# google-research/corenet

Hardware: AMD Instinct MI355X
Metric: voxels/sec fwd+bwd @128^3 (higher is better)
Workload: dtype bf16x3 (the convolutions of decoder stages 3-6 and the encoder's 3x3 convolutions -- forward of stages 4-5, data gradient of all -- multiply operands split into two bf16 terms: three bf16 MFMAs per product, fp32 accumulation, 16 mantissa bits, ~3e-6 relative per layer; tensors, everything else and t

## Files before the change

corenet_amd/_lib.py:

```python
from __future__ import annotations

import ctypes as C
import os
from typing import Optional

import torch as t

_HERE = os.path.dirname(os.path.abspath(__file__))
TOOLS_LIB_PATH = os.path.join(os.path.dirname(_HERE), "tools", "_build", "libcorenet_hip_tools.so")
PROBE_LIB_PATH = os.path.join(os.path.dirname(_HERE), "tools", "_build", "libcrn_probe.so")
LIB_PATH = os.environ.get("CORENET_HIP_LIB", TOOLS_LIB_PATH if os.environ.get("CRN_TOOLS_LIB") == "1" else
                          os.path.join(_HERE, "lib", "libcorenet_hip.so"))

c_i32p = C.POINTER(C.c_int32)
c_f32p = C.c_void_p
vp = C.c_void_p
i64 = C.c_int64
i32 = C.c_int
f32 = C.c_float
sz = C.c_size_t


class CrnTapBoxes(C.Structure):
  _fields_ = [("n_groups", C.c_int32), ("c_groups", C.c_int32), ("n_box", (C.c_int8 * 6) * 8),
# ... 42 lines not shown
    "crn_bf3_gather_image": [vp, vp, i32, vp, vp],
    "crn_convt_s2k7_fwd_bf3": [vp, i64, i32, i32, i32, i32, C.POINTER(CrnInTransform), vp, vp, vp, i64, i64, i32, vp],
    "crn_convt_s2k7_dgrad_bf3": [vp, i64, i64, i32, i32, i32, i32, i32, vp, vp, i64, i32, vp],
    "crn_convt_s2k7_c2_fwd_bf3": [vp, i64, i32, i32, i32, i32, C.POINTER(CrnInTransform), vp, vp, vp, i64, i64, i32, vp],
    "crn_convt_s2k7_c2_dgrad_bf3": [vp, i64, i64, i32, i32, i32, i32, i32, vp, vp, i64, i32, vp],
    "crn_convt_s2k7_wgrad_bf3": [vp, i64, i32, i32, i32, i32, C.POINTER(CrnInTransform), vp, i64, i64, i32, vp, i32, i32, vp, vp],
    "crn_convt_s2k7_ximage": [vp, i64, i32, i32, i32, i32, C.POINTER(CrnInTransform), vp, sz, vp],
    "crn_splitk_defer": [i32],
    "crn_splitk_reserve": [i64, vp],
    "crn_splitk_release": [vp],
    "crn_set_deterministic": [i32],
    "crn_roctx_push": [C.c_char_p],
    "crn_roctx_pop": [],
    "crn_comm_unique_id": [vp],
    "crn_comm_init": [vp, i32, i32, C.POINTER(vp)],
    "crn_comm_destroy": [vp],
    "crn_comm_info": [vp, C.POINTER(i32), C.POINTER(i32), C.POINTER(i32)],
    "crn_allreduce_f32": [vp, vp, i64, vp],
    "crn_broadcast_f32": [vp, vp, i64, i32, vp],
    "crn_conv_wgrad_1x1_bf3": [C.POINTER(CrnView), C.POINTER(CrnInTransform), C.POINTER(CrnView), vp, i32, i32, vp],
    "crn_conv_wgrad_2d_bf3": [C.POINTER(CrnView), C.POINTER(CrnInTransform), C.POINTER(CrnView), vp, i32, i32, i32, i32,
                              i32, i32, vp],
    "crn_conv2d_bf3": [C.POINTER(CrnView), C.POINTER(CrnInTransform), vp, i32, vp, i32, C.POINTER(CrnView),
                       i32, i32, i32, i32, i32, vp],
    "crn_copy_tiles_f32": [vp, vp, vp, vp, vp, i64, i32, vp],
    "crn_copy_mats_f32": [vp, vp, vp, i64, i32, vp],
    "crn_gather_f32": [vp, vp, vp, i64, vp],
    "crn_scatter_f32": [vp, vp, vp, i64, i32, vp],
    "crn_bias_grad": [vp, i32, i32, i64, i64, vp, i32, vp, sz, vp],
    "crn_batch_renorm_stats": [vp, i32, i32, i64, i64, i32, vp, vp, vp, vp, vp, f32, f32, i32,
                               vp, vp, vp, vp, sz, vp],
    "crn_batch_renorm_stats_tail": [vp, i32, i32, i64, i64, vp, vp, vp, vp, vp, f32, f32, i32, vp, vp, vp, vp, sz,
                                    vp, vp, vp, i64, vp, i64, vp, i64, i32, vp, i32, vp],
    "crn_batch_renorm_bwd_head": [vp, i64, vp, i64, vp, i64, vp, i64, vp, i64, i32, i32, i64, vp, vp, vp, vp, vp, i64,
                                  vp, vp, i32, vp, i32, vp, sz, vp, i32, vp],
    "crn_batch_renorm_bwd": [vp, i64, vp, i64, i32, i32, i64, i32, i32, vp, vp, vp, vp, vp, i64,
                             vp, vp, i32, vp, i32, vp, sz, vp],
    "crn_affine_add_relu": [vp, vp, vp, vp, vp, vp, i32, i32, i64, i64, i64, vp, i64, vp, i64, i32, vp],
    "crn_relu_bwd_add": [vp, vp, vp, i32, i32, i64, i64, i64, i64, vp, i64, vp],
    "crn_preprocess_caffe": [vp, i32, i32, i32, vp, vp],
    "crn_stem_conv_fwd": [vp, i32, i32, i32, vp, vp, vp, vp, sz, vp],
    "crn_stem_conv_wgrad": [vp, i32, i32, i32, vp, vp, vp],
    "crn_batch_renorm_finalize": [vp, i32, i32, C.c_double, vp, vp, vp, vp, vp, f32, f32, vp, vp, vp, vp],
    "crn_bn_relu_maxpool_fwd": [vp, vp, vp, i32, i32, i32, i32, vp, vp, vp],
    "crn_bn_relu_maxpool_bwd": [vp, vp, i32, i32, i32, i32, vp, vp],
    "crn_relu_mean_fwd": [vp, i32, i32, i64, i64, vp, vp],
    "crn_relu_mean_bwd": [vp, vp, i32, i32, i64, i64, vp, i64, i32, vp],
    "crn_linear_fwd": [vp, vp, vp, i32, i32, i32, vp, i32, vp],
    "crn_linear_bwd": [vp, vp, vp, i32, i32, i32, i32, vp, vp, vp, vp],
    "crn_stride2_gather": [vp, vp, i32, i32, i32, i32, i32, i32, vp],
    "crn_stride2_scatter": [vp, vp, i32, i32, i32, i32, i32, i32, vp],
    "crn_fill_offset_channels": [vp, i32, i64, i64, i32, vp, vp],
    "crn_decoder_inputs": [vp, vp, i32, i32, C.POINTER(C.c_float), vp, vp, vp],
    "crn_ray_sample_fwd": [vp, i64, i64, i64, i32, i32, i32, i32, vp, vp, vp, i64, i32, i32, i32, vp],
    "crn_ray_sample_bwd": [vp, i64, i32, i32, i32, i32, i32, vp, vp, vp, i64, i32, i32, i32, vp],
    "crn_ray_sample_fwd_idx": [vp, i64, i64, i64, i32, i32, i32, i32, vp, vp, vp, i64, i32, i32, i32, vp, vp],
    "crn_ray_project": [vp, vp, i32, i32, i32, i32, i32, i32, vp, vp],
    "crn_ray_sample_bwd_idx": [vp, i64, i32, i32, i32, i32, i32, vp, vp, i64, i32, i32, i32, vp],
    "crn_loss_fwd_bwd": [i32, vp, vp, vp, i32, i32, i64, vp, vp, f32, vp, sz, vp],
    "crn_argmax_confusion": [vp, vp, i32, i32, i64, vp, vp, vp],
    "crn_softmax_superres": [vp, i32, i32, i32, i32, i32, i32, vp, vp],
    "crn_adam_step": [vp, vp, vp, vp, i64, f32, f32, f32, f32, f32, i32, vp],
    "crn_adam_set_hyper": [vp, f32, f32, f32, f32, f32, i32, vp],
    "crn_adam_step_hyper": [vp, vp, vp, vp, i64, vp, vp],
    "crn_fill_voxels": [vp, vp, i32, i32, i32, i32, i32, vp, sz, vp],
    "crn_fill_voxels_strided": [vp, C.POINTER(i64), vp, C.POINTER(i64), i32, i32, i32, i32, i32, vp, sz, vp],
    "crn_fill_voxels_cpu": [vp, vp, i32, i32, i32, i32, i32, i32],
    "crn_marching_cubes_count": [vp, C.POINTER(i64), i32, i32, i32, i32, f32, vp, sz, vp, vp],
    "crn_marching_cubes_emit": [vp, C.POINTER(i64), i32, i32, i32, i32, f32, vp, vp, sz, vp, vp, vp, vp],
    "crn_marching_cubes_cpu": [vp, C.POINTER(i64), i32, i32, i32, i32, f32, vp, vp, vp, vp, vp, i32],
    "crn_box_filter": [vp, C.POINTER(i64), vp, i32, i32, i32, i32, i32, vp, sz, vp],
    "crn_box_filter_cpu": [vp, C.POINTER(i64), vp, i32, i32, i32, i32, i32, i32],
    "crn_render_bin": [vp, vp, i32, i32, i32, i32, i64, vp, vp, vp, vp],
    "crn_render_raster": [vp, vp, vp, vp, i32, vp, i32, i32, i32, i32, vp, vp, vp, vp, vp, vp],
    "crn_render_cpu": [vp, vp, vp, vp, i32, vp, i32, i32, i32, vp, i32],
    "crn_voxel_faces_count": [vp, i32, i32, i32, i32, vp, i32, vp, vp, vp, sz, vp, vp],
    "crn_voxel_faces_emit": [vp, i32, i32, i32, i32, vp, i32, vp, i32, vp, sz, vp, vp, vp, vp],
    "crn_voxel_faces_cpu": [vp, i32, i32, i32, i32, vp, i32, vp, vp, vp, i32, vp, vp, vp, vp, i32],
    "crn_voxelize_mesh": [vp, vp, i32, vp, i32, i32, i32, i32, i32, f32, i32, i32, vp, vp],
    "crn_batch_renorm_eval_affine": [vp, vp, vp, i32, f32, vp, vp, vp],
    "crn_transform_meshes": [vp, vp, i32, vp, i32, vp, vp],
    "crn_merge_labels": [vp, vp, vp, i32, i32, i32, i32, i32, vp, vp],
    "crn_zero_f32": [vp, i64, vp],
    "crn_add_i64": [vp, i32, i64, vp],
}
_SIZE_FNS = {
    "crn_batch_renorm_workspace_bytes": [i32],
    "crn_loss_workspace_bytes": [i32, i32],
    "crn_fill_voxels_workspace_bytes": [i32, i32, i32, i32],
    "crn_marching_cubes_workspace_bytes": [i32, i32, i32, i32],
    "crn_voxel_faces_workspace_bytes": [i32, i32, i32, i32],
    "crn_convt_s2k7_ximage_bytes": [i32, i32, i32, i32],
    "crn_stem_conv_parts": [i32, i32, i32],
}
_PTR_FNS = {
    "crn_loss_status_ptr": [vp, i32],
}
TOOL_SYMBOLS = ["crn_bf3_debug_stamps", "crn_e2d_debug_stamps", "crn_pw_debug_stamps"]
ALL_SYMBOLS = list(_SIGS) + list(_SIZE_FNS) + list(_PTR_FNS) + ["crn_version"]


class _Lib:
  def __init__(self, path: str):
    if not os.path.exists(path):
      raise ImportError(
          f"{path} not found: build it with `python -m corenet_amd.build` "
          "(corenet_amd has no CPU or eager-PyTorch fallback).")
    self.path = path
    self.cdll = C.CDLL(path)
    for name, sig in _SIGS.items():
      fn = getattr(self.cdll, name)
      fn.argtypes = sig
      fn.restype = C.c_int
      setattr(self, "_" + name, fn)
    for name, sig in _SIZE_FNS.items():
      fn = getattr(self.cdll, name)
      fn.argtypes = sig
      fn.restype = C.c_size_t
      setattr(self, name, fn)
    for name, sig in _PTR_FNS.items():
      fn = getattr(self.cdll, name)
      fn.argtypes = sig
      fn.restype = C.c_void_p
      setattr(self, name, fn)
    self.cdll.crn_version.restype = C.c_char_p

  def version(self) -> str:
    return self.cdll.crn_version().decode()

  def __getattr__(self, name):
    if name.startswith("crn_"):
      fn = object.__getattribute__(self, "_" + name)

      def call(*args):
        rc = fn(*args)
        if rc != 0:
          raise HipError(f"{name} failed with status {rc}")
      setattr(self, name, call)
      return call
    raise AttributeError(name)


_lib: Optional[_Lib] = None


def lib() -> _Lib:
  global _lib
  if _lib is None:
    _lib = _Lib(LIB_PATH)
  return _lib


def ptr(x: Optional[t.Tensor]) -> Optional[int]:
  if x is None:
    return None
  return x.data_ptr()


import threading

_tls = threading.local()


def stream() -> int:
  s = getattr(_tls, "stream", None)
  if s is not None:
# ... 49 lines not shown
```

corenet_amd/backend.py:

```python
from __future__ import annotations

import ctypes as C
from typing import Optional

import torch as t

from corenet_amd import _lib
from corenet_amd._lib import CrnInTransform, CrnView, ptr
from corenet_amd.views import View

_DTYPE_CODE = {t.float32: 0, t.uint8: 1, t.int32: 2, t.float64: 3, t.int64: 4, t.int16: 5, t.int8: 6}


def _cview(v: View) -> CrnView:
  base = v.storage.data_ptr() + 4 * (v.offset - v.storage.storage_offset())
  c = v.__dict__.get("_crn")
  if c is None or c[0] != base:
    c = (base, CrnView(base, v.B, v.C, v.D, v.H, v.W, v.sB, v.sC, ptr(v.chan_off), v.sD, v.sH, v.sW))
    object.__setattr__(v, "_crn", c)
  return c[1]


class Transform:
  __slots__ = ("scale", "shift", "pre_relu", "post_relu")

  def __init__(self, scale: t.Tensor, shift: t.Tensor, pre_relu=False, post_relu=False):
    self.scale, self.shift = scale, shift
    self.pre_relu, self.post_relu = bool(pre_relu), bool(post_relu)


def _ctr(tr: Optional[Transform]):
  if tr is None:
    return None
  return C.byref(CrnInTransform(ptr(tr.scale), ptr(tr.shift), int(tr.pre_relu), int(tr.post_relu)))


_TAPBOXES = {}


def _ctapboxes(boxes):
  if not boxes or not (boxes[0] or boxes[1]):
    return None
  key = (tuple(boxes[0]), tuple(boxes[1]))
  tb = _TAPBOXES.get(key)
  if tb is None:
    tb = _lib.CrnTapBoxes()
    tb.n_groups, tb.c_groups = len(key[0]), len(key[1])
    for g, bx in enumerate(key[0]):
      for i, v in enumerate(bx): tb.n_box[g][i] = v
    for g, bx in enumerate(key[1]):
      for i, v in enumerate(bx): tb.c_box[g][i] = v
    _TAPBOXES[key] = tb
  return C.cast(C.pointer(tb), C.c_void_p)


class HipBackend:
  name = "hip"

  def __init__(self):
    self.lib = _lib.lib()
    self._ws = {}
    self._deterministic = False

  def workspace(self, key: str, nbytes: int, device) -> t.Tensor:
    w = self._ws.get((key, str(device)))
    if w is None or w.numel() < nbytes:
      w = t.empty(max(nbytes, 1), dtype=t.uint8, device=device)
      self._ws[(key, str(device))] = w
    return w

  def _bn_ws(self, Cn: int, device):
    n = self.lib.crn_batch_renorm_workspace_bytes(Cn)
    return self.workspace("bn@%x" % _lib.stream(), n, device), n

  def conv_fwd(self, x: View, tr: Optional[Transform], w: t.Tensor, npad: int,
               bias: Optional[t.Tensor], bias_sB: int, y: View, window, pad_lo,
               splits: int = 1, accumulate: bool = False, boxes=None, math: str = "fp32", wslab=None):
    if math == "bf16x3" and wslab is not None:
      self.lib.crn_conv_fwd_bf3_slabs(C.byref(_cview(x)), _ctr(tr), ptr(wslab), npad, ptr(bias), bias_sB,
                                      C.byref(_cview(y)), window[0], window[1], window[2],
                                      pad_lo[0], pad_lo[1], pad_lo[2], int(accumulate), _ctapboxes(boxes), _lib.stream())
      return
    if math == "bf16x3":
      self.lib.crn_conv_fwd_bf3(C.byref(_cview(x)), _ctr(tr), ptr(w), npad, ptr(bias), bias_sB,
                                C.byref(_cview(y)), window[0], window[1], window[2],
                                pad_lo[0], pad_lo[1], pad_lo[2], int(accumulate), _ctapboxes(boxes), _lib.stream())
      return
    self.lib.crn_conv_fwd(C.byref(_cview(x)), _ctr(tr), ptr(w), npad, ptr(bias), bias_sB,
                          C.byref(_cview(y)), window[0], window[1], window[2],
                          pad_lo[0], pad_lo[1], pad_lo[2], splits, int(accumulate), _ctapboxes(boxes),
                          _lib.stream())

  def conv_fwd_stats(self, x: View, tr: Optional[Transform], wslab: t.Tensor, npad: int, bias, bias_sB: int, y: View, window,
                     pad_lo, boxes, Cn: int, pre_relu: bool) -> int:
    ws, n = self._bn_ws(Cn, y.storage.device)
    parts = C.c_int(0)
    self.lib.crn_conv_fwd_bf3_slabs_stats(C.byref(_cview(x)), _ctr(tr), ptr(wslab), npad, ptr(bias), bias_sB,
                                          C.byref(_cview(y)), window[0], window[1], window[2], pad_lo[0], pad_lo[1], pad_lo[2],
                                          0, _ctapboxes(boxes), int(pre_relu), ptr(ws), n, C.byref(parts), _lib.stream())
    return parts.value

  def conv_dgrad_bn_bwd(self, dyv: View, wslab: t.Tensor, npad: int, gv: View, g: t.Tensor, window, pad_lo, boxes,
                        x, sB_x, B, Cn, S, pre_relu, gamma, scale, shift, saved, dx, sB_dx, dgamma, dbeta,
                        dsum=None, ndsum=0) -> bool:
    ws, n = self._bn_ws(Cn, x.device)
    f = _lib.CrnBnBwdFuse(ptr(x), sB_x, ptr(saved), int(pre_relu), ptr(ws), n, ptr(dsum), int(ndsum), 0)
    self.lib.crn_conv_fwd_bf3_slabs_bnbwd(C.byref(_cview(dyv)), None, ptr(wslab), npad, None, 0, C.byref(_cview(gv)),
                                          window[0], window[1], window[2], pad_lo[0], pad_lo[1], pad_lo[2], 0,
                                          _ctapboxes(boxes), C.byref(f), _lib.stream())
    if f.nparts <= 0:
      return False
    self.lib.crn_batch_renorm_bwd_apply(ptr(x), sB_x, ptr(g), Cn * S, B, Cn, S, int(pre_relu), ptr(gamma),
                                        ptr(scale), ptr(shift), ptr(saved), ptr(dx), sB_dx, ptr(dgamma), ptr(dbeta),
                                        0, ptr(dsum), int(ndsum), ptr(ws), n, f.nparts, _lib.stream())
    return True

  def splitk_defer(self, on: bool = True):
    self.lib.crn_splitk_defer(int(on))

  def set_deterministic(self, on: bool = True):
    self.lib.crn_set_deterministic(int(on))
    self._deterministic = bool(on)

  def splitk_reserve(self, stream: t.cuda.Stream, floats: int = 0):
    self.lib.crn_splitk_reserve(int(floats), stream.cuda_stream)

  def splitk_release(self, stream: t.cuda.Stream):
    self.lib.crn_splitk_release(stream.cuda_stream)
    for k in [k for k in self._ws if k[0] == "bn@%x" % stream.cuda_stream]:
      del self._ws[k]

  def bf3_operands(self, packed: t.Tensor, table, out: t.Tensor):
    desc, blocks = table
    self.lib.crn_bf3_operands(ptr(packed), ptr(desc), desc.shape[0], blocks, ptr(out), _lib.stream())

  def bf3_gather_image(self, src: t.Tensor, table: t.Tensor, out: t.Tensor, host_table=None):
    self.lib.crn_bf3_gather_image(ptr(src), ptr(table), table.shape[0], ptr(out), _lib.stream())

  def convt_par_fwd(self, x: t.Tensor, tr: Optional[Transform], wimg: t.Tensor, bias: Optional[t.Tensor], y: t.Tensor, cout: int,
                    host_table=None, resident: bool = False):
    B, cin, D, H, W = x.shape
    assert cin == 16 and x[0].is_contiguous() and y[0].is_contiguous() and tuple(y.shape[2:]) == (2 * D, 2 * H, 2 * W)
    fn = self.lib.crn_convt_s2k7_c2_fwd_bf3 if resident else self.lib.crn_convt_s2k7_fwd_bf3
    fn(ptr(x), x.stride(0), B, D, H, W, _ctr(tr), ptr(wimg), ptr(bias), ptr(y), y.stride(0), y.stride(1), cout, _lib.stream())

  def convt_par_dgrad(self, dy: t.Tensor, cout: int, wimg: t.Tensor, dx: t.Tensor, accumulate: bool = False, host_table=None,
                      resident: bool = False):
    B, cin, D, H, W = dx.shape
    assert cin == 16 and dx[0].is_contiguous() and dy[0].is_contiguous() and tuple(dy.shape[2:]) == (2 * D, 2 * H, 2 * W)
    fn = self.lib.crn_convt_s2k7_c2_dgrad_bf3 if resident else self.lib.crn_convt_s2k7_dgrad_bf3
    fn(ptr(dy), dy.stride(0), dy.stride(1), cout, B, D, H, W, ptr(wimg), ptr(dx), dx.stride(0), int(accumulate), _lib.stream())

  def conv2d_bf3(self, x: View, tr: Optional[Transform], wop: t.Tensor, npad: int, bias: Optional[t.Tensor],
                 bias_sB: int, y: View, window, pad_lo, accumulate: bool = False):
    assert window[0] == 1 and pad_lo[0] == 0
    self.lib.crn_conv2d_bf3(C.byref(_cview(x)), _ctr(tr), ptr(wop), npad, ptr(bias), bias_sB, C.byref(_cview(y)),
                            window[1], window[2], pad_lo[1], pad_lo[2], int(accumulate), _lib.stream())

  def convt_ximage(self, x: t.Tensor, tr: Optional[Transform], img: Optional[t.Tensor] = None) -> Optional[t.Tensor]:
    if self._deterministic:
      return None
    B, cin, D, H, W = x.shape
    assert cin == 16 and x[0].is_contiguous()
    nb = self.lib.crn_convt_s2k7_ximage_bytes(B, D, H, W)
    if img is None or img.numel() < nb:
      img = t.empty(nb, dtype=t.uint8, device=x.device)
    self.lib.crn_convt_s2k7_ximage(ptr(x), x.stride(0), B, D, H, W, _ctr(tr), ptr(img), nb, _lib.stream())
    return img

  def conv_wgrad(self, x: View, tr: Optional[Transform], dy: View, dw: t.Tensor, npad: int,
                 window, pad_lo, zero_first: bool = True, boxes=None, math: str = "fp32", ximg: Optional[t.Tensor] = None):
    if math == "bf16x3_1x1":
      self.lib.crn_conv_wgrad_1x1_bf3(C.byref(_cview(x)), _ctr(tr), C.byref(_cview(dy)), ptr(dw), npad, int(zero_first),
                                      _lib.stream())
# ... 126 lines not shown
  def relu_mean_bwd(self, x_pre, davg, B, Cn, S, sB, dx, sB_dx, accumulate=False):
    self.lib.crn_relu_mean_bwd(ptr(x_pre), ptr(davg), B, Cn, S, sB, ptr(dx), sB_dx, int(accumulate),
                               _lib.stream())

  def linear_fwd(self, x, w, bias, B, K, N, y, ldy):
    self.lib.crn_linear_fwd(ptr(x), ptr(w), ptr(bias), B, K, N, ptr(y), ldy, _lib.stream())

  def linear_bwd(self, x, w, dy, lddy, B, K, N, dx, dw, db):
    self.lib.crn_linear_bwd(ptr(x), ptr(w), ptr(dy), lddy, B, K, N, ptr(dx), ptr(dw), ptr(db),
                            _lib.stream())

  def stride2_gather(self, x, y):
    B, Cn, h, w = y.shape
    self.lib.crn_stride2_gather(ptr(x), ptr(y), B, Cn, h, w, x.shape[2], x.shape[3], _lib.stream())

  def stride2_scatter(self, dy, dx):
    B, Cn, h, w = dy.shape
    self.lib.crn_stride2_scatter(ptr(dy), ptr(dx), B, Cn, h, w, dx.shape[2], dx.shape[3], _lib.stream())

  def decoder_inputs(self, v2s, offset, scales, layer_mats, offset_out):
    n = len(scales)
    arr = (C.c_float * n)(*[float(v) for v in scales])
    self.lib.crn_decoder_inputs(ptr(v2s), ptr(offset), v2s.shape[0], n, arr, ptr(layer_mats), ptr(offset_out), _lib.stream())

  def fill_offset_channels(self, x, B, sB, S, c0, offset):
    self.lib.crn_fill_offset_channels(ptr(x), B, sB, S, c0, ptr(offset), _lib.stream())

  def ray_sample_fwd(self, fmap, map_sB, B, Cn, h, w, matrix, offset, out, out_sB, D, H, W,
                     map_sC=None, map_sP=1):
    self.lib.crn_ray_sample_fwd(ptr(fmap), map_sB, h * w if map_sC is None else map_sC, map_sP, B, Cn, h, w,
                                ptr(matrix), ptr(offset), ptr(out), out_sB, D, H, W, _lib.stream())

  def ray_sample_bwd(self, dout, dout_sB, B, Cn, D, H, W, matrix, offset, dmap, dmap_sB, h, w,
                     zero_first=True):
    self.lib.crn_ray_sample_bwd(ptr(dout), dout_sB, B, Cn, D, H, W, ptr(matrix), ptr(offset),
                                ptr(dmap), dmap_sB, h, w, int(zero_first), _lib.stream())

  def ray_sample_fwd_idx(self, fmap, map_sB, B, Cn, h, w, matrix, offset, out, out_sB, D, H, W, idx,
                         map_sC=None, map_sP=1):
    self.lib.crn_ray_sample_fwd_idx(ptr(fmap), map_sB, h * w if map_sC is None else map_sC, map_sP, B, Cn, h, w,
                                    ptr(matrix), ptr(offset), ptr(out), out_sB, D, H, W, ptr(idx), _lib.stream())

  def ray_project(self, matrix, offset, B, D, H, W, h, w, idx):
    self.lib.crn_ray_project(ptr(matrix), ptr(offset), B, D, H, W, h, w, ptr(idx), _lib.stream())

  def ray_sample_bwd_idx(self, dout, dout_sB, B, Cn, D, H, W, idx, dmap, dmap_sB, h, w, zero_first=True):
    self.lib.crn_ray_sample_bwd_idx(ptr(dout), dout_sB, B, Cn, D, H, W, ptr(idx), ptr(dmap), dmap_sB, h, w,
                                    int(zero_first), _lib.stream())

  def loss_fwd_bwd(self, kind, logits, gt_i32, B, Cn, S, loss, dlogits, grad_scale=1.0, weights=None):
    n = self.lib.crn_loss_workspace_bytes(B, Cn)
    ws = self.workspace("loss", n, logits.device)
    self.lib.crn_loss_fwd_bwd(kind, ptr(logits), ptr(gt_i32), ptr(weights), B, Cn, S, ptr(loss), ptr(dlogits),
                              grad_scale, ptr(ws), n, _lib.stream())

  def loss_labels_in_range(self, B, Cn, device) -> bool:
    n = self.lib.crn_loss_workspace_bytes(B, Cn)
    ws = self.workspace("loss", n, device)
    off = self.lib.crn_loss_status_ptr(ptr(ws), B) - ws.data_ptr()
    return int(ws[off:off + 4].view(t.int32)) == 0

  def softmax_superres(self, logits, m, B, Cn, D, H, W, out):
    self.lib.crn_softmax_superres(ptr(logits), m, B, Cn, D, H, W, ptr(out), _lib.stream())

  def argmax_confusion(self, logits, gt_i32, B, Cn, S, labels, cm):
    self.lib.crn_argmax_confusion(ptr(logits), ptr(gt_i32), B, Cn, S, ptr(labels), ptr(cm), _lib.stream())

  def adam_step(self, p, g, m, v, n, lr, b1, b2, eps, grad_scale, step):
    self.lib.crn_adam_step(ptr(p), ptr(g), ptr(m), ptr(v), n, lr, b1, b2, eps, grad_scale, step,
                           _lib.stream())

  def adam_set_hyper(self, hyper, lr, b1, b2, eps, grad_scale, step):
    self.lib.crn_adam_set_hyper(ptr(hyper), lr, b1, b2, eps, grad_scale, step, _lib.stream())

  def adam_step_hyper(self, p, g, m, v, n, hyper):
    self.lib.crn_adam_step_hyper(ptr(p), ptr(g), ptr(m), ptr(v), n, ptr(hyper), _lib.stream())

  def add_i64(self, p, n, v):
    self.lib.crn_add_i64(ptr(p), n, v, _lib.stream())

  def zero(self, x: t.Tensor):
    self.lib.crn_zero_f32(ptr(x), x.numel(), _lib.stream())

  def fill_voxels(self, grid: t.Tensor, out: t.Tensor):
    N, D, H, W = grid.shape
    n = self.lib.crn_fill_voxels_workspace_bytes(N, D, H, W)
    ws = self.workspace("fill", n, grid.device)
    if grid.is_contiguous() and out.is_contiguous():
      self.lib.crn_fill_voxels(ptr(grid), ptr(out), _DTYPE_CODE[grid.dtype], N, D, H, W, ptr(ws), n,
                               _lib.stream())
    else:
      gs = (C.c_int64 * 4)(*grid.stride())
      os_ = (C.c_int64 * 4)(*out.stride())
      self.lib.crn_fill_voxels_strided(ptr(grid), gs, ptr(out), os_, _DTYPE_CODE[grid.dtype], N, D, H, W,
                                       ptr(ws), n, _lib.stream())

  def marching_cubes_count(self, grid: t.Tensor, level: float, counts: t.Tensor):
    N, D, H, W = grid.shape
    n = self.lib.crn_marching_cubes_workspace_bytes(N, D, H, W)
    ws = self.workspace("mc", n, grid.device)
    st = (C.c_int64 * 4)(*grid.stride())
    self.lib.crn_marching_cubes_count(ptr(grid), st, N, D, H, W, float(level), ptr(ws), n, ptr(counts), _lib.stream())

  def marching_cubes_emit(self, grid: t.Tensor, level: float, matrices: Optional[t.Tensor], vertices: t.Tensor,
                          normals: t.Tensor, faces: t.Tensor):
    N, D, H, W = grid.shape
    n = self.lib.crn_marching_cubes_workspace_bytes(N, D, H, W)
    ws = self.workspace("mc", n, grid.device)
    st = (C.c_int64 * 4)(*grid.stride())
    self.lib.crn_marching_cubes_emit(ptr(grid), st, N, D, H, W, float(level), ptr(matrices), ptr(ws), n, ptr(vertices),
                                     ptr(normals), ptr(faces), _lib.stream())

  def box_filter(self, grid: t.Tensor, k: int, out: t.Tensor):
    N, D, H, W = grid.shape
    n = 4 * grid.numel()
    ws = self.workspace("box", n, grid.device)
    st = (C.c_int64 * 4)(*grid.stride())
    self.lib.crn_box_filter(ptr(grid), st, ptr(out), N, D, H, W, int(k), ptr(ws), n, _lib.stream())

  def voxelize_mesh(self, tri, tri_mesh, view2voxel, M, D, H, W, sub_side, mult, conservative,
                    depth_mult, grid):
    self.lib.crn_voxelize_mesh(ptr(tri), ptr(tri_mesh), tri.shape[0], ptr(view2voxel), M, D, H, W,
                               sub_side, float(mult), int(conservative), depth_mult, ptr(grid),
                               _lib.stream())

  def transform_meshes(self, triangles, tri_mesh, mesh_matrix, out):
    self.lib.crn_transform_meshes(ptr(triangles), ptr(tri_mesh), triangles.shape[0], ptr(mesh_matrix),
                                  mesh_matrix.shape[0], ptr(out), _lib.stream())

  def merge_labels(self, meshes_grid, scene_start, labels, B, D, H, W, sub_grid, out):
    self.lib.crn_merge_labels(ptr(meshes_grid), ptr(scene_start), ptr(labels), B, D, H, W,
                              int(sub_grid), ptr(out), _lib.stream())


_default: Optional[HipBackend] = None


def default_backend() -> HipBackend:
  global _default
  if _default is None:
    _default = HipBackend()
  return _default
```

corenet_amd/csrc/conv_e2d.hip:

```cpp
#include "conv_kernels.h"
#include <algorithm>
#include <cstdlib>

namespace {
using namespace crnk;

typedef __bf16 bf16x8 __attribute__((ext_vector_type(8)));

struct E2dGeom {
  crnView x, y;
  crnInTransform tr;
  const void* wop;
  const float* bias;
  int bias_sB;
  int ntn;
  int nblk;
  int ph, pw;
  int tilesH, tilesW;
  int nchunks, chunks_per_split;
  int tab;
  int mode;
  int dbg;
  long long* stamps;
};
// ... 268 lines not shown
        const bf16x8 wl = __builtin_bit_cast(bf16x8, bl[s]);
        bf16x8 nh[4], nl[4];
        if (s + 1 < KS && !(g.dbg & 32)) {
          const int cbl = (s + 1) / T, t = (s + 1) % T;
          const int toff = cbl * 4 * PS + (t / KW) * PW + (t % KW);
#pragma unroll
          for (int ms = 0; ms < 4; ++ms) { nh[ms] = Ahi[aoff[ms] + toff]; nl[ms] = Alo[aoff[ms] + toff]; }
        }
        __builtin_amdgcn_sched_barrier(0);
        if (!(g.dbg & 4)) {
#pragma unroll
        for (int ms = 0; ms < 4; ++ms) acc[ms] = __builtin_amdgcn_mfma_f32_16x16x32_bf16(ah[ms], wh, acc[ms], 0, 0, 0);
#pragma unroll
        for (int ms = 0; ms < 4; ++ms) acx[ms] = __builtin_amdgcn_mfma_f32_16x16x32_bf16(ah[ms], wl, acx[ms], 0, 0, 0);
#pragma unroll
        for (int ms = 0; ms < 4; ++ms) acx[ms] = __builtin_amdgcn_mfma_f32_16x16x32_bf16(al[ms], wh, acx[ms], 0, 0, 0);
        }
        b_issue(chunk + 1, s, (g.dbg & 64) ? kOOB : step_oob(chunk + 1, s), bh[s], bl[s]);
        if (s + 1 < KS && !(g.dbg & 32)) {
#pragma unroll
          for (int ms = 0; ms < 4; ++ms) { ah[ms] = nh[ms]; al[ms] = nl[ms]; }
        }
      }
      mark(4 + 2 * (chunk - cbeg));
      patch_wait();
      mark(5 + 2 * (chunk - cbeg));
      if (chunk + 1 < cend) {
        bf16x8* Nhi = Abuf + (buf ^ 1) * 2 * PLANE;
        patch_commit(chunk + 1, Nhi, Nhi + PLANE);
      }
      __syncthreads();
    }
  }

#pragma unroll
  for (int s = 0; s < KS; ++s) asm volatile("s_waitcnt vmcnt(0)" : "+v"(bh[s]), "+v"(bl[s]));
  if constexpr (T == 9) {
#pragma unroll
    for (int i = 0; i < 16; i += 8)
      asm volatile("s_waitcnt vmcnt(0)"
                   : "+v"(pf[i]), "+v"(pf[i + 1]), "+v"(pf[i + 2]), "+v"(pf[i + 3]), "+v"(pf[i + 4]), "+v"(pf[i + 5]),
                     "+v"(pf[i + 6]), "+v"(pf[i + 7]));
  } else {
#pragma unroll
    for (int i = 0; i < 8; ++i) asm volatile("s_waitcnt vmcnt(0)" : "+v"(pv[i]));
  }

  mark(30);
#pragma unroll
  for (int ms = 0; ms < 4; ++ms) acc[ms] += acx[ms];
  const int n = ntile * 16 + i16;
  if (n >= g.y.C || (g.dbg & 8)) return;
  const float bsv = (g.bias && split == 0) ? g.bias[(int64_t)b * g.bias_sB + n] : 0.f;
  float* yb = g.y.base + (int64_t)(g.mode == 3 ? split * g.x.B + b : b) * g.y.sB + (int64_t)n * g.y.sC;
  if constexpr (T == 9) {
#pragma unroll
    for (int ms = 0; ms < 4; ++ms) {
      const int rr = 4 * kk;
      const int oh = h0 + ms * (16 / TW) + rr / TW, ow = w0 + rr % TW;
      float* dst = yb + (int64_t)oh * g.y.sH + ow;
      f32x4 v = acc[ms] + bsv;
      if (g.mode == 1) v += *reinterpret_cast<const f32x4*>(dst);
      *reinterpret_cast<f32x4*>(dst) = v;
    }
  } else {
#pragma unroll
    for (int r = 0; r < 4; ++r) {
      float* dst = yb + p0 + 16 * kk + 4 * r;
      f32x4 v = (f32x4){acc[0][r], acc[1][r], acc[2][r], acc[3][r]} + bsv;
      if (g.mode == 1) v += *reinterpret_cast<const f32x4*>(dst);
      *reinterpret_cast<f32x4*>(dst) = v;
    }
  }
  mark(31);
}

struct Wg1Geom {
  const float* x; const float* dy; float* dw;
  const float* scale; const float* shift;
  int pre_relu, post_relu;
  long long xsB, dsB;
  int C, N, Npad, S;
  int ksteps, ksteps_per_block;
};

__global__ __launch_bounds__(256, 2) void wgrad1x1_bf3_kernel(Wg1Geom g) {
  crn_kernargs_now(g.x, g.dy, g.dw, g.scale, g.shift, g.pre_relu, g.post_relu, g.xsB, g.dsB, g.C, g.N, g.Npad, g.S,
                   g.ksteps, g.ksteps_per_block);
  __shared__ __attribute__((aligned(16))) f32x4 red[4][8][64];
  const int tid = threadIdx.x, lane = tid & 63;
  const int wave = __builtin_amdgcn_readfirstlane(tid >> 6);
  const int i16 = lane & 15, kk = lane >> 4;
  const int c0 = blockIdx.x * 64, n0 = blockIdx.y * 32;
  const int kbeg = blockIdx.z * g.ksteps_per_block, kend = min(kbeg + g.ksteps_per_block, g.ksteps);
  unsigned arow[4], brow[2];
  float sc[4], sh[4];
  const bool has_tr = g.scale != nullptr;
#pragma unroll
  for (int mt = 0; mt < 4; ++mt) {
    const int c = c0 + 16 * mt + i16;
    arow[mt] = c < g.C ? (unsigned)c * (unsigned)g.S * 4u : kOOB;
    sc[mt] = (has_tr && c < g.C) ? g.scale[c] : 1.f;
    sh[mt] = (has_tr && c < g.C) ? g.shift[c] : 0.f;
  }
#pragma unroll
  for (int nt = 0; nt < 2; ++nt) {
    const int n = n0 + 16 * nt + i16;
    brow[nt] = n < g.N ? (unsigned)n * (unsigned)g.S * 4u : kOOB;
  }
  f32x4 acc[4][2];
#pragma unroll
  for (int mt = 0; mt < 4; ++mt)
#pragma unroll
    for (int nt = 0; nt < 2; ++nt) acc[mt][nt] = (f32x4){0.f, 0.f, 0.f, 0.f};

  f32x4 ra[4][2], rb[2][2];
  auto issue = [&](int step) {
    const bool live = step < kend;
    const int pos = step * 32, b = live ? pos / g.S : 0, s = pos - b * g.S;
    const crn_rsrc xrs = make_rsrc(g.x + (long long)b * g.xsB);
    const crn_rsrc drs = make_rsrc(g.dy + (long long)b * g.dsB);
    const unsigned koff = (unsigned)(s + 8 * kk) * 4u, oob = live ? 0u : kOOB;
#pragma unroll
    for (int mt = 0; mt < 4; ++mt) {
      crn_bload4(ra[mt][0], xrs, (arow[mt] + koff) | oob);
      crn_bload4(ra[mt][1], xrs, (arow[mt] + koff + 16u) | oob);
    }
#pragma unroll
    for (int nt = 0; nt < 2; ++nt) {
      crn_bload4(rb[nt][0], drs, (brow[nt] + koff) | oob);
      crn_bload4(rb[nt][1], drs, (brow[nt] + koff + 16u) | oob);
    }
  };
  auto wait_all = [&]() {
#pragma unroll
    for (int mt = 0; mt < 4; ++mt) asm volatile("s_waitcnt vmcnt(0)" : "+v"(ra[mt][0]), "+v"(ra[mt][1]));
#pragma unroll
    for (int nt = 0; nt < 2; ++nt) asm volatile("s_waitcnt vmcnt(0)" : "+v"(rb[nt][0]), "+v"(rb[nt][1]));
  };
  int step = kbeg + wave;
  issue(step);
  for (; step < kend; step += 4) {
    wait_all();
    bf16x8 ah[4], al[4], bh[2], bl[2];
#pragma unroll
    for (int mt = 0; mt < 4; ++mt) {
      float v[8];
#pragma unroll
      for (int j = 0; j < 8; ++j) {
        float a = ra[mt][j >> 2][j & 3];
        if (has_tr) {
          if (g.pre_relu) a = fmaxf(a, 0.f);
          a = a * sc[mt] + sh[mt];
          if (g.post_relu) a = fmaxf(a, 0.f);
        }
        v[j] = a;
      }
      if (has_tr && arow[mt] == kOOB) {
#pragma unroll
        for (int j = 0; j < 8; ++j) v[j] = 0.f;
      }
      split8(v, ah[mt], al[mt]);
    }
#pragma unroll
    for (int nt = 0; nt < 2; ++nt) {
      float v[8];
#pragma unroll
      for (int j = 0; j < 8; ++j) v[j] = rb[nt][j >> 2][j & 3];
      split8(v, bh[nt], bl[nt]);
    }
    issue(step + 4);
#pragma unroll
    for (int nt = 0; nt < 2; ++nt) {
#pragma unroll
      for (int mt = 0; mt < 4; ++mt) acc[mt][nt] = __builtin_amdgcn_mfma_f32_16x16x32_bf16(ah[mt], bh[nt], acc[mt][nt], 0, 0, 0);
#pragma unroll
      for (int mt = 0; mt < 4; ++mt) acc[mt][nt] = __builtin_amdgcn_mfma_f32_16x16x32_bf16(ah[mt], bl[nt], acc[mt][nt], 0, 0, 0);
#pragma unroll
      for (int mt = 0; mt < 4; ++mt) acc[mt][nt] = __builtin_amdgcn_mfma_f32_16x16x32_bf16(al[mt], bh[nt], acc[mt][nt], 0, 0, 0);
    }
  }
  wait_all();
#pragma unroll
  for (int mt = 0; mt < 4; ++mt)
#pragma unroll
    for (int nt = 0; nt < 2; ++nt) red[wave][mt * 2 + nt][lane] = acc[mt][nt];
  __syncthreads();
#pragma unroll
  for (int q = 0; q < 2; ++q) {
    const int tile = wave * 2 + q;
    const f32x4 v = red[0][tile][lane] + red[1][tile][lane] + red[2][tile][lane] + red[3][tile][lane];
    const int mt = tile >> 1, nt = tile & 1;
    const int n = n0 + 16 * nt + i16;
#pragma unroll
    for (int r = 0; r < 4; ++r) {
      const int c = c0 + 16 * mt + 4 * kk + r;
      if (c < g.C && n < g.N) atomicAdd(g.dw + (long long)c * g.Npad + n, v[r]);
    }
  }
}

struct Wg3Geom {
  const float* x; const float* dy; float* dw;
  const float* scale; const float* shift;
  int pre_relu, post_relu;
  long long xsB, dsB;
  int C, N, Npad, S, H, W;
  int ksteps, ksteps_per_block;
};

__global__ __launch_bounds__(256, 2) void wgrad3x3_bf3_kernel(Wg3Geom g) {
  crn_kernargs_now(g.x, g.dy, g.dw, g.scale, g.shift, g.pre_relu, g.post_relu, g.xsB, g.dsB, g.C, g.N, g.Npad, g.S, g.H,
                   g.W, g.ksteps, g.ksteps_per_block);
  __shared__ __attribute__((aligned(16))) f32x4 red[4][12][64];
  const int tid = threadIdx.x, lane = tid & 63;
  const int wave = __builtin_amdgcn_readfirstlane(tid >> 6);
  const int i16 = lane & 15, kk = lane >> 4;
  const int q0 = blockIdx.x * 32, n0 = blockIdx.y * 32;
  const int kbeg = blockIdx.z * g.ksteps_per_block, kend = min(kbeg + g.ksteps_per_block, g.ksteps);
  const bool has_tr = g.scale != nullptr;
  unsigned arow[2], brow[2];
  int dzh[2];
  float sc[2], sh[2];
#pragma unroll
  for (int qt = 0; qt < 2; ++qt) {
    const int q = q0 + 16 * qt + i16, c = q / 3;
    dzh[qt] = q - 3 * c - 1;
    arow[qt] = c < g.C ? (unsigned)c * (unsigned)g.S * 4u : kOOB;
    sc[qt] = (has_tr && c < g.C) ? g.scale[c] : 1.f;
    sh[qt] = (has_tr && c < g.C) ? g.shift[c] : 0.f;
  }
#pragma unroll
  for (int nt = 0; nt < 2; ++nt) {
    const int n = n0 + 16 * nt + i16;
    brow[nt] = n < g.N ? (unsigned)n * (unsigned)g.S * 4u : kOOB;
  }
  f32x4 acc[6][2];
#pragma unroll
  for (int mt = 0; mt < 6; ++mt)
#pragma unroll
    for (int nt = 0; nt < 2; ++nt) acc[mt][nt] = (f32x4){0.f, 0.f, 0.f, 0.f};

  f32x4 ra[2][2], rb[2][2];
  float el[2], er[2];
  unsigned vmask = 0;
  auto issue = [&](int step) {
    const bool live = step < kend;
    const int pos = step * 32, b = live ? pos / g.S : 0, s = pos - b * g.S + 8 * kk;
    const int h = s / g.W, w0 = s - h * g.W;
    const crn_rsrc xrs = make_rsrc(g.x + (long long)b * g.xsB);
    const crn_rsrc drs = make_rsrc(g.dy + (long long)b * g.dsB);
    vmask = 0;
#pragma unroll
    for (int qt = 0; qt < 2; ++qt) {
      const int hh = h + dzh[qt];
      const bool ok = live && arow[qt] != kOOB && hh >= 0 && hh < g.H;
      const bool okl = ok && w0 > 0, okr = ok && w0 + 8 < g.W;
      const unsigned off = arow[qt] + (unsigned)(s + dzh[qt] * g.W) * 4u;
      vmask |= (ok ? 1u : 0u) << qt | (okl ? 1u : 0u) << (2 + qt) | (okr ? 1u : 0u) << (4 + qt);
      crn_bload4(ra[qt][0], xrs, ok ? off : kOOB);
      crn_bload4(ra[qt][1], xrs, ok ? off + 16u : kOOB);
      crn_bload(el[qt], xrs, okl ? off - 4u : kOOB);
      crn_bload(er[qt], xrs, okr ? off + 32u : kOOB);
    }
    const unsigned koff = (unsigned)s * 4u, oob = live ? 0u : kOOB;
// ... 123 lines not shown
  const bool armed = crn_splitk_take_armed();
  { const int rcf = crn_splitk_flush(st); if (rcf != CRN_OK) return rcf; }
  E2dGeom g{};
  g.x = *x; g.y = *y;
  if (tr) g.tr = *tr; else g.tr = crnInTransform{nullptr, nullptr, 0, 0};
  g.wop = wop; g.bias = bias; g.bias_sB = bias_sB;
  g.ntn = Npad / 16; g.nblk = x->C / 32; g.ph = ph; g.pw = pw;
#ifdef CRN_TOOLS
  static const bool want_stamps = getenv("CRN_E2D_DBG") && (atoi(getenv("CRN_E2D_DBG")) & 16);
  if (want_stamps) {
    if (!g_stamps) CRN_HIP(hipMalloc(&g_stamps, 32 * sizeof(long long)));
    g.stamps = g_stamps;
    g.dbg = 16;
  }
#endif
  int TW = 16, CB = 1;
  int64_t tiles;
  if (k3) {
    if (x->D != 1 || ph < 0 || ph > 2 || pw < 0 || pw > 2) return CRN_EINVAL;
    TW = (x->W % 16 == 0) ? 16 : 8;
    const int TH = 64 / TW;
    if (x->W % TW || x->H % TH) return CRN_EINVAL;
    g.tilesW = x->W / TW; g.tilesH = x->H / TH;
    tiles = (int64_t)g.tilesW * g.tilesH;
    g.nchunks = g.nblk;
  } else {
    if (S % 64) return CRN_EINVAL;
    CB = 4;
    g.tilesW = (int)(S / 64); g.tilesH = 1;
    tiles = g.tilesW;
    g.nchunks = (g.nblk + CB - 1) / CB;
  }
  const int64_t base_blocks = tiles * x->B * (y->C / 64);
  constexpr int kFill = 256;
  int splits = 1;
  while (base_blocks * splits < kFill && splits * 2 <= g.nchunks && splits < 16) splits *= 2;
  g.chunks_per_split = (g.nchunks + splits - 1) / splits;
  splits = (g.nchunks + g.chunks_per_split - 1) / g.chunks_per_split;
  g.tab = g.tr.scale ? g.chunks_per_split * CB * 32 : 0;
  crnView yreal = *y;
  const float* scratch = nullptr;
  if (splits > 1) {
    float* sc = crn_splitk_scratch((size_t)splits * x->B * y->C * S, st);
    if (!sc) return CRN_ENOMEM;
    scratch = sc;
    g.y.base = sc; g.y.sC = S; g.y.sB = (int64_t)y->C * S; g.y.sH = x->W; g.y.sD = x->H * x->W;
    g.mode = 3;
  } else {
    g.mode = accumulate ? 1 : 0;
  }
  const size_t plane_bytes = (size_t)(k3 ? 4 * (128 + 4) : 16 * (64 + 4)) * 16;
  const size_t lds = (size_t)g.tab * 8 + 4 * plane_bytes;
  if (lds > 160 * 1024) return CRN_EINVAL;
  const dim3 grid((unsigned)(tiles * x->B), (unsigned)(y->C / 64), (unsigned)splits);
  int rc;
  if (k1) rc = launch_e2d<1, 4, 16>(g, grid, lds, st);
  else if (TW == 16) rc = launch_e2d<9, 1, 16>(g, grid, lds, st);
  else rc = launch_e2d<9, 1, 8>(g, grid, lds, st);
  if (rc == CRN_OK && splits > 1) {
    if (armed && !accumulate && yreal.sB == (int64_t)yreal.C * S) {
      crn_splitk_set_pending(yreal, scratch, splits, st);
      return rc;
    }
    rc = crn_splitk_reduce(yreal, scratch, splits, accumulate, st);
  }
  return rc;
}

#ifdef CRN_TOOLS
extern "C" int crn_e2d_debug_stamps(long long* out32) {
  if (!g_stamps) return CRN_EINVAL;
  CRN_HIP(hipDeviceSynchronize());
  CRN_HIP(hipMemcpy(out32, g_stamps, 32 * sizeof(long long), hipMemcpyDeviceToHost));
  return CRN_OK;
}
#endif

extern "C" int crn_conv_wgrad_1x1_bf3(const crnView* x, const crnInTransform* tr, const crnView* dy, float* dw, int Npad,
                                      int zero_first, crnStream stream) {
  CRN_ENTRY(stream);
  return crn_conv_wgrad_2d_bf3(x, tr, dy, dw, Npad, 1, 1, 0, 0, zero_first, stream);
}

extern "C" int crn_conv_wgrad_2d_bf3(const crnView* x, const crnInTransform* tr, const crnView* dy, float* dw, int Npad,
                                     int kh, int kw, int ph, int pw, int zero_first, crnStream stream) {
  CRN_ENTRY(stream);
  if (!x || !dy || !dw || Npad <= 0 || (Npad & 15) || x->B != dy->B || dy->C > Npad) return CRN_EINVAL;
  if (!dense_2d(*x) || !dense_2d(*dy)) return CRN_EINVAL;
  if (x->D != dy->D || x->H != dy->H || x->W != dy->W) return CRN_EINVAL;
  const int64_t S = (int64_t)x->D * x->H * x->W;
  if (S % 32 || x->sC != S || dy->sC != S) return CRN_EINVAL;
  if (S * x->C * 4 >= ((int64_t)1 << 31) || S * dy->C * 4 >= ((int64_t)1 << 31)) return CRN_EINVAL;
  hipStream_t st = (hipStream_t)stream;
  if (kh == 3 && kw == 3) {
    if (ph != 1 || pw != 1 || x->D != 1 || (x->W & 7)) return CRN_EINVAL;
    if (zero_first) CRN_HIP(hipMemsetAsync(dw, 0, (size_t)x->C * 9 * Npad * 4, st));
    Wg3Geom g{};
    g.x = x->base; g.dy = dy->base; g.dw = dw;
    g.scale = tr ? tr->scale : nullptr; g.shift = tr ? tr->shift : nullptr;
    g.pre_relu = tr ? tr->pre_relu : 0; g.post_relu = tr ? tr->post_relu : 0;
    g.xsB = x->sB; g.dsB = dy->sB; g.C = x->C; g.N = dy->C; g.Npad = Npad; g.S = (int)S; g.H = x->H; g.W = x->W;
    g.ksteps = (int)((int64_t)x->B * S / 32);
    const int tiles = crn_cdiv(3 * x->C, 32) * crn_cdiv(dy->C, 32);
    constexpr int kFill3 = 512;
    int splits = std::max(1, std::min(g.ksteps / 8, crn_cdiv(kFill3, tiles)));
    if (crn_deterministic()) splits = 1;
    g.ksteps_per_block = crn_cdiv(g.ksteps, splits);
    splits = crn_cdiv(g.ksteps, g.ksteps_per_block);
    const dim3 grid((unsigned)crn_cdiv(3 * x->C, 32), (unsigned)crn_cdiv(dy->C, 32), (unsigned)splits);
    hipLaunchKernelGGL(wgrad3x3_bf3_kernel, grid, dim3(256), 0, st, g);
    CRN_CHECK_LAUNCH();
    return CRN_OK;
  }
  if (kh != 1 || kw != 1 || ph || pw) return CRN_EINVAL;
  if (zero_first) CRN_HIP(hipMemsetAsync(dw, 0, (size_t)x->C * Npad * 4, st));
  Wg1Geom g{};
  g.x = x->base; g.dy = dy->base; g.dw = dw;
  g.scale = tr ? tr->scale : nullptr; g.shift = tr ? tr->shift : nullptr;
  g.pre_relu = tr ? tr->pre_relu : 0; g.post_relu = tr ? tr->post_relu : 0;
  g.xsB = x->sB; g.dsB = dy->sB; g.C = x->C; g.N = dy->C; g.Npad = Npad; g.S = (int)S;
  g.ksteps = (int)((int64_t)x->B * S / 32);
  const int tiles = crn_cdiv(x->C, 64) * crn_cdiv(dy->C, 32);
  constexpr int kFill = 512;
  int splits = std::max(1, std::min(g.ksteps / 8, crn_cdiv(kFill, tiles)));
  if (crn_deterministic()) splits = 1;
  g.ksteps_per_block = crn_cdiv(g.ksteps, splits);
  splits = crn_cdiv(g.ksteps, g.ksteps_per_block);
  const dim3 grid((unsigned)crn_cdiv(x->C, 64), (unsigned)crn_cdiv(dy->C, 32), (unsigned)splits);
  hipLaunchKernelGGL(wgrad1x1_bf3_kernel, grid, dim3(256), 0, st, g);
  CRN_CHECK_LAUNCH();
  return CRN_OK;
}
```

corenet_amd/csrc/conv_igemm.hip:

```cpp
#include "conv_kernels.h"
#include <algorithm>
#include <mutex>
#include <cstring>
#include <cstdio>
#include <cstdlib>
#include <vector>

namespace {
using namespace crnk;

struct PwGeom {
  const float* x; float* y; const float* w; const float* bias;
  crnInTransform tr;
  int B, C, N, Npad, S;
  int64_t xsB, ysB;
  int64_t ysC, ysP;
  int bias_sB, mode;
  int splits, cps;
  long long* stamps;
};

constexpr int kPwTab = 2048;
template <int NS>
__global__ __launch_bounds__(256) void pointwise_fwd_kernel(PwGeom g) {
  constexpr int BM = 64, BN = NS * 16, KC = 64, SA = BM + 16, SB = BN + 16;
  constexpr int NRA = KC / 16;
  __shared__ __attribute__((aligned(16))) float ldsA[KC * SA];
  __shared__ __attribute__((aligned(16))) float ldsB[KC * SB];
  crn_kernargs_now(g.x, g.y, g.w, g.bias, g.tr.scale, g.tr.shift, g.tr.pre_relu, g.tr.post_relu, g.B, g.C, g.N, g.Npad,
                   g.S, g.xsB, g.ysB, g.ysC, g.ysP, g.bias_sB, g.mode, g.splits, g.cps);
  const long long t_entry = (long long)__builtin_amdgcn_s_memtime();
  const long long r_entry = (long long)__builtin_amdgcn_s_memrealtime();
  const int tid = threadIdx.x, lane = tid & 63, wave = tid >> 6;
  const int i16 = lane & 15, kk = lane >> 4;
  const int m0 = blockIdx.x * BM, n0 = blockIdx.y * BN;
  const bool stamp = g.stamps && blockIdx.x == 0 && blockIdx.y == 0 && blockIdx.z == 0 && tid == 0;
  int nmark = 0;
  auto mark = [&]() { if (stamp && nmark < 30) g.stamps[nmark] = (long long)__builtin_amdgcn_s_memtime() - t_entry; ++nmark; };
  mark();
  const int split = blockIdx.z / g.B, b = blockIdx.z - split * g.B;
  const int cbeg = split * g.cps, cend = min(g.C, cbeg + g.cps);
  const float* xb = g.x + (int64_t)b * g.xsB;
  const int ka = tid >> 4, ca = (tid & 15) * 4;
  constexpr int BQ = BN / 4, BROWS = 256 / BQ, NRB = KC / BROWS;
  const int kb = tid / BQ, cb = (tid % BQ) * 4;
  const bool a_ok = (m0 + ca) < g.S;
  const bool b_ok = (n0 + cb) < g.Npad;
  extern __shared__ float pw_tables[];
  const bool has_tr = g.tr.scale != nullptr;
  float* tsc = pw_tables; float* tsh = pw_tables + g.cps;
  constexpr unsigned kOOBo = 0x80000000u;
  constexpr int NL = NRA + NRB;
  const crn_rsrc xrs = crnk::make_rsrc(xb);
  const crn_rsrc wrs = crnk::make_rsrc(g.w);
  f32x4 ra[2][NRA], rb[2][NRB];
  auto issue = [&](int c0, f32x4 (&pa_)[NRA], f32x4 (&pb_)[NRB]) {
#pragma unroll
    for (int q = 0; q < NRA; ++q) {
      const int c_a = c0 + ka + q * 16;
      const unsigned off = (a_ok && c_a < cend) ? (unsigned)(c_a * g.S + m0 + ca) * 4u : kOOBo;
      crnk::crn_bload4(pa_[q], xrs, off);
    }
#pragma unroll
    for (int q = 0; q < NRB; ++q) {
      const int c_b = c0 + kb + q * BROWS;
      const unsigned off = (b_ok && c_b < cend) ? (unsigned)(c_b * g.Npad + n0 + cb) * 4u : kOOBo;
      crnk::crn_bload4(pb_[q], wrs, off);
    }
  };
  auto wait_slot = [&](f32x4 (&pa_)[NRA], f32x4 (&pb_)[NRB]) {
#pragma unroll
    for (int q = 0; q < NRA; ++q) asm volatile("s_waitcnt vmcnt(%1)" : "+v"(pa_[q]) : "n"(NL));
#pragma unroll
    for (int q = 0; q < NRB; ++q) asm volatile("s_waitcnt vmcnt(%1)" : "+v"(pb_[q]) : "n"(NL));
  };
  auto xform = [&](f32x4 v, int c) -> f32x4 {
    if (has_tr && a_ok && c < cend) {
      const float sc = tsc[c - cbeg], sh = tsh[c - cbeg];
#pragma unroll
      for (int i = 0; i < 4; ++i) {
        float t = v[i];
        if (g.tr.pre_relu) t = fmaxf(t, 0.f);
        t = t * sc + sh;
        if (g.tr.post_relu) t = fmaxf(t, 0.f);
        v[i] = t;
      }
    }
    return v;
  };
  f32x4 acc[NS];
#pragma unroll
  for (int ns = 0; ns < NS; ++ns) acc[ns] = (f32x4){0.f, 0.f, 0.f, 0.f};
  issue(cbeg, ra[0], rb[0]);
  issue(cbeg + KC, ra[1], rb[1]);
  mark();
  if (has_tr)
    for (int c = tid; c < cend - cbeg; c += 256) { tsc[c] = g.tr.scale[cbeg + c]; tsh[c] = g.tr.shift[cbeg + c]; }
  auto step = [&](int c0, f32x4 (&pa_)[NRA], f32x4 (&pb_)[NRB]) {
    wait_slot(pa_, pb_);
    mark();
    __syncthreads();
#pragma unroll
    for (int q = 0; q < NRA; ++q) *reinterpret_cast<f32x4*>(ldsA + (ka + q * 16) * SA + ca) = xform(pa_[q], c0 + ka + q * 16);
#pragma unroll
    for (int q = 0; q < NRB; ++q) *reinterpret_cast<f32x4*>(ldsB + (kb + q * BROWS) * SB + cb) = pb_[q];
    __syncthreads();
    mark();
    issue(c0 + 2 * KC, pa_, pb_);
    const float* pa = ldsA + kk * SA + wave * 16 + i16;
    const float* pb = ldsB + kk * SB + i16;
#pragma unroll
    for (int ks = 0; ks < KC / 4; ++ks) {
      const float a = pa[ks * 4 * SA];
      float bv[NS];
#pragma unroll
      for (int ns = 0; ns < NS; ++ns) bv[ns] = pb[ks * 4 * SB + ns * 16];
#pragma unroll
      for (int ns = 0; ns < NS; ++ns) acc[ns] = __builtin_amdgcn_mfma_f32_16x16x4f32(a, bv[ns], acc[ns], 0, 0, 0);
    }
    mark();
  };
  for (int c0 = cbeg; c0 < cend; c0 += 2 * KC) {
    step(c0, ra[0], rb[0]);
    if (c0 + KC < cend) step(c0 + KC, ra[1], rb[1]);
  }
#pragma unroll
  for (int sl = 0; sl < 2; ++sl) {
#pragma unroll
    for (int q = 0; q < NRA; ++q) asm volatile("s_waitcnt vmcnt(0)" : "+v"(ra[sl][q]));
#pragma unroll
    for (int q = 0; q < NRB; ++q) asm volatile("s_waitcnt vmcnt(0)" : "+v"(rb[sl][q]));
  }
  const int m = m0 + wave * 16 + kk * 4;
  if (m < g.S) {
#pragma unroll
    for (int ns = 0; ns < NS; ++ns) {
      const int n = n0 + ns * 16 + i16;
      if (n < g.N) {
        const float bsv = (g.bias && split == 0) ? g.bias[(int64_t)b * g.bias_sB + n] : 0.f;
        float* dst = g.y + (int64_t)(split * g.B + b) * g.ysB + (int64_t)n * g.ysC + (int64_t)m * g.ysP;
        f32x4 v = acc[ns] + bsv;
        if (g.ysP == 1) {
          if (g.mode == 1) v += *reinterpret_cast<const f32x4*>(dst);
          *reinterpret_cast<f32x4*>(dst) = v;
        } else {
#pragma unroll
          for (int i = 0; i < 4; ++i) dst[i * g.ysP] = g.mode == 1 ? dst[i * g.ysP] + v[i] : v[i];
        }
      }
    }
  }
  if (stamp) {
    g.stamps[31] = (long long)__builtin_amdgcn_s_memtime() - t_entry;
    g.stamps[30] = (long long)__builtin_amdgcn_s_memrealtime() - r_entry;
  }
}

constexpr int kDenseB = 8;
__global__ __launch_bounds__(256) void dense_cols_kernel(const float* x, int64_t xsB, int64_t xsC, crnInTransform tr,
                                                         const float* w, int Npad, int N, int C, int B,
                                                         const float* bias, int bias_sB, float* y, int64_t ysB,
                                                         int64_t ysC, int accumulate) {
  extern __shared__ float xs[];
  __shared__ float red[3][kDenseB][64];
  const int lane = threadIdx.x & 63, wave = threadIdx.x >> 6;
  const int n = blockIdx.x * 64 + lane;
  const int cq = (C + 3) >> 2, cbeg = wave * cq, cend = min(C, cbeg + cq);
  const bool col = n < N;
  float wv[32];
#pragma unroll
  for (int u = 0; u < 32; ++u) wv[u] = (col && cbeg + u < cend) ? w[(int64_t)(cbeg + u) * Npad + n] : 0.f;
  for (int i = threadIdx.x; i < B * C; i += blockDim.x) {
    const int b = i / C, c = i - b * C;
    float v = x[b * xsB + c * xsC];
    if (tr.scale) {
      if (tr.pre_relu) v = fmaxf(v, 0.f);
      v = v * tr.scale[c] + tr.shift[c];
      if (tr.post_relu) v = fmaxf(v, 0.f);
    }
    xs[i] = v;
  }
  __syncthreads();
  float acc[kDenseB];
#pragma unroll
  for (int b = 0; b < kDenseB; ++b) acc[b] = 0.f;
  for (int c = cbeg; c < cend; c += 32) {
    if (c > cbeg) {
#pragma unroll
      for (int u = 0; u < 32; ++u) wv[u] = (col && c + u < cend) ? w[(int64_t)(c + u) * Npad + n] : 0.f;
    }
#pragma unroll
    for (int u = 0; u < 32; ++u)
#pragma unroll
      for (int b = 0; b < kDenseB; ++b)
        if (b < B && c + u < cend) acc[b] += xs[b * C + c + u] * wv[u];
  }
  if (wave) {
#pragma unroll
    for (int b = 0; b < kDenseB; ++b) red[wave - 1][b][lane] = acc[b];
// ... 256 lines not shown
  p.active = false;
  (void)st;
  int cur = -1;
  CRN_HIP(hipGetDevice(&cur));
  if (cur != p.device) CRN_HIP(hipSetDevice(p.device));
  const int rc = crn_splitk_reduce(p.y, p.scratch, p.splits, 0, p.stream);
  if (cur != p.device) CRN_HIP(hipSetDevice(cur));
  return rc;
}
void crn_splitk_set_pending(const crnView& y, const float* scratch, int splits, hipStream_t st) {
  CrnSplitPending& p = crn_splitk_pending();
  p.active = true; p.y = y; p.scratch = scratch; p.splits = splits; p.stream = st;
  if (hipGetDevice(&p.device) != hipSuccess) p.device = 0;
}
extern "C" int crn_splitk_defer(int on) {
  crn_splitk_pending().armed = on != 0;
  return CRN_OK;
}
float* crn_splitk_scratch(size_t floats, hipStream_t st) { return splitk_scratch(floats, st); }
extern "C" int crn_splitk_reserve(int64_t floats, crnStream stream) {
  int dev = 0;
  CRN_HIP(hipGetDevice(&dev));
  size_t want = floats > 0 ? (size_t)floats : 0;
  if (!want) {
    std::lock_guard<std::mutex> lock(g_sk_mu);
    for (int i = 0; i < kSkSlots; ++i)
      if (g_sk_slots[i].used && g_sk_slots[i].dev == dev) want = std::max(want, g_sk_slots[i].cap);
  }
  {
    std::lock_guard<std::mutex> lock(g_sk_mu);
    SkSlot* sl = nullptr;
    for (int i = 0; i < kSkSlots && !sl; ++i)
      if (g_sk_slots[i].used && g_sk_slots[i].dev == dev && g_sk_slots[i].st == (hipStream_t)stream) sl = &g_sk_slots[i];
    for (int i = 0; i < kSkSlots && !sl; ++i)
      if (!g_sk_slots[i].used) { g_sk_slots[i] = SkSlot{dev, (hipStream_t)stream, nullptr, 0, true, false, nullptr}; sl = &g_sk_slots[i]; }
    if (!sl) return CRN_ENOMEM;
    sl->pinned = true;
  }
  if (!want) return CRN_OK;
  return splitk_scratch(want, (hipStream_t)stream) ? CRN_OK : CRN_ENOMEM;
}
extern "C" int crn_splitk_release(crnStream stream) {
  int dev = 0;
  CRN_HIP(hipGetDevice(&dev));
  std::lock_guard<std::mutex> lock(g_sk_mu);
  for (int i = 0; i < kSkSlots; ++i) {
    SkSlot& sl = g_sk_slots[i];
    if (sl.used && sl.dev == dev && sl.st == (hipStream_t)stream) {
      if (sl.buf) CRN_HIP(hipFree(sl.buf));
      if (sl.retired) {
        for (float* b : *sl.retired) (void)hipFree(b);
        delete sl.retired;
      }
      sl = SkSlot{};
    }
  }
  return CRN_OK;
}
int crn_splitk_reduce(const crnView& y, const float* scratch, int splits, int accumulate, hipStream_t st) {
  const int64_t ytot = (int64_t)y.B * y.C * y.D * y.H * y.W;
  const int64_t per_b = (int64_t)y.C * y.D * y.H * y.W;
  if (plain_view(y) && (per_b & 3) == 0 && (((uintptr_t)scratch) & 15) == 0) {
    const int64_t total4 = ytot / 4;
    hipLaunchKernelGGL(splitk_reduce_plain_kernel, dim3((unsigned)std::min<int64_t>(crn_cdiv(total4, 256), 4096)), dim3(256),
                       0, st, y.base, y.sB, scratch, per_b / 4, total4, splits, accumulate);
    CRN_CHECK_LAUNCH();
    return CRN_OK;
  }
  hipLaunchKernelGGL(splitk_reduce_kernel, dim3((unsigned)std::min<int64_t>(crn_cdiv(ytot, 256), 4096)), dim3(256), 0, st,
                     y, scratch, splits, accumulate);
  CRN_CHECK_LAUNCH();
  return CRN_OK;
}

static long long* g_pw_stamps = nullptr;
#ifdef CRN_TOOLS
extern "C" int crn_pw_debug_stamps(long long* out32) {
  if (!g_pw_stamps) return CRN_EINVAL;
  CRN_HIP(hipDeviceSynchronize());
  CRN_HIP(hipMemcpy(out32, g_pw_stamps, 32 * sizeof(long long), hipMemcpyDeviceToHost));
  return CRN_OK;
}
#endif
extern "C" int crn_conv_fwd(const crnView* x, const crnInTransform* tr, const float* w, int Npad,
                            const float* bias, int bias_sB, const crnView* y,
                            int kd, int kh, int kw, int pd, int ph, int pw,
                            int splits, int accumulate, const crnTapBoxes* boxes, crnStream stream) {
  if (boxes && (boxes->n_groups < 0 || boxes->n_groups > 8 || boxes->c_groups < 0 || boxes->c_groups > 8)) return CRN_EINVAL;
  if (!x || !y || !w || Npad <= 0 || (Npad & 15) || x->B != y->B || kd < 1 || kh < 1 || kw < 1)
    return CRN_EINVAL;
  if (y->C > Npad) return CRN_EINVAL;
  hipStream_t st = (hipStream_t)stream;
  const bool armed = crn_splitk_take_armed();
  { const int rcf = crn_splitk_flush(st); if (rcf != CRN_OK) return rcf; }
  const int64_t Sx = (int64_t)x->D * x->H * x->W;
  if (kd * kh * kw == 1 && pd == 0 && ph == 0 && pw == 0 && splits <= 1 && one_position(*x) && one_position(*y) &&
      x->B <= kDenseB) {
    const crnInTransform trv = tr ? *tr : crnInTransform{nullptr, nullptr, 0, 0};
    if (y->C >= 1024 && x->C <= 2048) {
      hipLaunchKernelGGL(dense_cols_kernel, dim3((unsigned)crn_cdiv(y->C, 64)), dim3(256), (size_t)x->B * x->C * 4, st,
                         x->base, x->sB, x->sC, trv, w, Npad, y->C, x->C, x->B, bias, bias_sB, y->base, y->sB, y->sC,
                         accumulate);
      CRN_CHECK_LAUNCH();
      return CRN_OK;
    }
    if (y->C <= 256 && !trv.scale && x->C >= 1024) {
      const int zs = (y->sC == 1 && y->sB >= y->C && !crn_deterministic()) ? std::max(1, std::min(16, x->C / 2048)) : 1;
      if (zs > 1 && !accumulate)
        CRN_HIP(hipMemset2DAsync(y->base, (size_t)y->sB * 4, 0, (size_t)y->C * 4, (size_t)x->B, st));
      hipLaunchKernelGGL(dense_rows_kernel, dim3((unsigned)crn_cdiv(y->C, 8), (unsigned)x->B, (unsigned)zs), dim3(256), 0, st,
                         x->base, x->sB, x->sC, w, Npad, y->C, x->C, bias, bias_sB, y->base, y->sB, y->sC, accumulate,
                         crn_cdiv(x->C, zs));
      CRN_CHECK_LAUNCH();
      return CRN_OK;
    }
  }
  if (kd * kh * kw == 1 && pd == 0 && ph == 0 && pw == 0 && splits <= 1 && plain_view(*x) && flat_out_view(*y) &&
      Sx == (int64_t)y->D * y->H * y->W && (Sx & 3) == 0 && (((uintptr_t)w) & 15) == 0 &&
      (int64_t)x->C * Sx * 4 < ((int64_t)1 << 31) && (int64_t)x->C * Npad * 4 < ((int64_t)1 << 31) &&
      (!tr || !tr->scale || x->C <= kPwTab)) {
    PwGeom p{};
    p.x = x->base; p.y = y->base; p.w = w; p.bias = bias;
    p.tr = tr ? *tr : crnInTransform{nullptr, nullptr, 0, 0};
    p.B = x->B; p.C = x->C; p.N = y->C; p.Npad = Npad; p.S = (int)Sx;
    p.xsB = x->sB; p.ysB = y->sB; p.bias_sB = bias_sB; p.mode = accumulate ? 1 : 0;
    p.ysC = y->sC; p.ysP = y->sW;
    p.splits = 1; p.cps = (x->C + 63) & ~63;
    constexpr int BNh = 32, pw_blocks = 256, pw_fill = 512, pw_minc = 128;
    const int64_t blocks = crn_cdiv(Sx, 64) * crn_cdiv(y->C, BNh) * (int64_t)x->B;
    const int64_t ytot = (int64_t)y->B * y->C * Sx;
    float* scratch = nullptr;
    if (splits < 1 && blocks < pw_blocks && x->C >= 2 * pw_minc) {
      int sp = (int)std::min<int64_t>(std::min<int64_t>(x->C / pw_minc, 16), crn_cdiv(pw_fill, blocks));
      if (sp > 1) {
        p.cps = (crn_cdiv(x->C, sp) + 31) & ~31;
        sp = crn_cdiv(x->C, p.cps);
        if (sp > 1 && (scratch = splitk_scratch((size_t)sp * ytot, st)) != nullptr) {
          p.splits = sp; p.y = scratch; p.ysB = (int64_t)y->C * Sx; p.ysC = Sx; p.ysP = 1; p.mode = 0;
        } else {
          p.cps = (x->C + 31) & ~31;
        }
      }
    }
#ifdef CRN_TOOLS
    static const bool want_stamps = getenv("CRN_PW_STAMPS") != nullptr;
#else
    constexpr bool want_stamps = false;
#endif
    static long long* pw_stamps = nullptr;
    if (want_stamps) {
      if (!pw_stamps) CRN_HIP(hipMalloc(&pw_stamps, 32 * sizeof(long long)));
      CRN_HIP(hipMemsetAsync(pw_stamps, 0, 32 * sizeof(long long), st));
      p.stamps = pw_stamps;
      g_pw_stamps = pw_stamps;
    }
    dim3 grid((unsigned)crn_cdiv(Sx, 64), (unsigned)crn_cdiv(y->C, BNh), (unsigned)(x->B * p.splits));
    const size_t tab_bytes = p.tr.scale ? (size_t)2 * p.cps * sizeof(float) : 0;
    hipLaunchKernelGGL(pointwise_fwd_kernel<2>, grid, dim3(256), tab_bytes, st, p);
    CRN_CHECK_LAUNCH();
    if (p.splits > 1) {
      if (armed && !accumulate && plain_view(*y) && y->sB == (int64_t)y->C * Sx) {
        crn_splitk_set_pending(*y, scratch, p.splits, st);
        return CRN_OK;
      }
      return crn_splitk_reduce(*y, scratch, p.splits, accumulate, st);
    }
    return CRN_OK;
  }
  static const int kM[4] = {8, 4, 2, 1};
  static const int kN[3] = {4, 2, 1};
  const int xmode = vec_view(*x) ? 1 : ((x->sW == 2 && (x->W & 1) == 0) ? 2 : 0);
  g_stage_unit = xmode == 2 ? 2 : 4;
  const int lead = xmode == 1 ? vec_lead(pw) : (xmode == 2 ? ((pw % 2) + 2) % 2 : -1);
  constexpr double kSplitPenalty = 20000.0;
  constexpr int kSplitFill = 512;
  FwdCfg best{}; bool have = false; double best_cost = 1e300; int best_splits = 1;
  for (int mi = 0; mi < 4; ++mi)
    for (int ni = 0; ni < 3; ++ni) {
      if (kN[ni] > 1 && kN[ni] * 16 > Npad) continue;
      if (kM[mi] * kN[ni] > 8) continue;
      FwdCfg c;
      if (!fwd_cfg(kM[mi], kN[ni], y->B, x->C, Npad, y->D, y->H, y->W, kd, kh, kw, lead, &c)) continue;
      const int T = kd * kh * kw, nchunks = crn_cdiv(x->C, c.CC), NB = kN[ni] * 16;
      const int TD = c.tsd, TH = c.tsh * c.mh, TW = c.tsw * c.mw;
      const double patch = (double)c.CC * (TD + kd - 1) * (TH + kh - 1) * patch_width(TW, kw, lead);
      const double slots = (lead >= 0 ? patch / g_stage_unit / 256 * (g_stage_unit == 4 ? 450.0 : 400.0) : patch / 256 * 350.0) +
                           (double)c.CC * T * NB / 4 / 256 * 300.0;
      const double chunk_work = (double)kM[mi] * kN[ni] * (c.CC / 4) * T * 32.0 * 1.3 + slots;
      for (int sp = 1; sp <= (splits < 1 ? std::min(nchunks, 64) : 1); sp *= 2) {
        if (sp > 1 && c.blocks * (sp / 2) >= kSplitFill) break;
        const int cps = crn_cdiv(nchunks, sp);
        const double bpc = std::max(1.0, std::ceil((double)c.blocks * sp / 256.0));
        double cost = bpc * cps * chunk_work + cps * std::ceil(bpc / 2.0) * 9000.0 + (sp > 1 ? kSplitPenalty : 0.0);
        if (cost < best_cost) { best_cost = cost; best = c; have = true; best_splits = sp; }
      }
    }
  bool forced = false;
  int xvec = lead >= 0 ? xmode : 0;
  if (!have && xvec) {
    xvec = 0;
    for (int mi = 0; mi < 4 && !have; ++mi) {
      FwdCfg c;
      if (fwd_cfg(kM[mi], 1, y->B, x->C, Npad, y->D, y->H, y->W, kd, kh, kw, -1, &c)) { best = c; have = true; forced = true; }
    }
  }
  if (!have) return CRN_EINVAL;
  ConvGeom g{};
  g.x = *x; g.y = *y;
  if (tr) g.tr = *tr; else g.tr = crnInTransform{nullptr, nullptr, 0, 0};
  g.w = w; g.bias = bias; g.Npad = Npad; g.bias_sB = bias_sB;
  g.lead = xvec ? lead : 0;
  g.kd = kd; g.kh = kh; g.kw = kw; g.pd = pd; g.ph = ph; g.pw = pw + g.lead; g.T = kd * kh * kw;
  g.mw = best.mw; g.mh = best.mh; g.nsh = best.tsh; g.nsw = best.tsw;
  g.TD = best.tsd; g.TH = best.tsh * best.mh; g.TW = best.tsw * best.mw;
  g.PD = g.TD + kd - 1; g.PH = g.TH + kh - 1; g.PW = patch_width(g.TW, kw, xvec ? lead : -1);
  g.PS = g.PD * g.PH * g.PW; g.PSP = pad16mod32(g.PS);
  g.tilesD = crn_cdiv(y->D, g.TD); g.tilesH = crn_cdiv(y->H, g.TH); g.tilesW = crn_cdiv(y->W, g.TW);
  const int NSUB = best.NSUB, CC = best.CC;
  g.CC = CC; g.WSP = pad16mod32(g.T * NSUB * 16);
  g.nchunks = crn_cdiv(x->C, CC);
  if (splits < 1) {
    splits = forced ? (best.blocks >= 192 ? 1 : (int)std::min<int64_t>(std::min(g.nchunks, 16), crn_cdiv(256, best.blocks)))
                    : best_splits;
  }
  if (splits > g.nchunks) splits = g.nchunks;
  g.chunks_per_split = crn_cdiv(g.nchunks, splits);
  splits = crn_cdiv(g.nchunks, g.chunks_per_split);
  g.mode = splits > 1 ? 2 : (accumulate ? 1 : 0);
  g.lg2 = ilog2_ceil(g.PH * g.PW); g.npass = xvec ? 0 : stage_passes(CC * g.PD, g.PH * g.PW);
  g.magic_PW = magic20(g.PW); g.magic_PD = magic20(g.PD); g.magic_T = magic20(g.T);
  if (xvec) {
    g.plu = g.PH * g.PW / g_stage_unit; g.pw4 = g.PW / g_stage_unit; g.nunits = CC * g.PD * g.plu;
    g.magic_PLU = magic20(g.plu); g.magic_PW4 = magic20(g.pw4);
  }
  const crnView yreal = *y;
  const int64_t ytot = (int64_t)y->B * y->C * y->D * y->H * y->W;
  float* scratch = g.mode == 2 ? splitk_scratch((size_t)splits * ytot, st) : nullptr;
  if (scratch) {
    g.mode = 3;
    const int64_t S = (int64_t)y->D * y->H * y->W;
    g.y.base = scratch; g.y.chan_off = nullptr;
    g.y.sW = 1; g.y.sH = y->W; g.y.sD = y->H * y->W; g.y.sC = S; g.y.sB = (int64_t)y->C * S;
  }
  y = &g.y;
  if (g.mode == 2 && !accumulate) {
    hipLaunchKernelGGL(zero_view_kernel, dim3((unsigned)std::min<int64_t>(crn_cdiv(ytot, 256), 4096)),
                       dim3(256), 0, st, yreal);
    CRN_CHECK_LAUNCH();
  }
  dim3 grid((unsigned)(g.tilesD * g.tilesH * g.tilesW * y->B), (unsigned)crn_cdiv(Npad, NSUB * 16),
            (unsigned)splits);
// ... 73 lines not shown
    return true;
  };
  auto search = [&]() {
    static const int kTD[4] = {4, 3, 2, 1};
    static const int kTH[6] = {16, 8, 6, 4, 2, 1};
    for (int tdi = 0; tdi < 4; ++tdi)
      for (int thi = 0; thi < 6; ++thi)
        for (int NSUB = 4; NSUB >= 1; NSUB >>= 1)
          for (int RSUB = 8; RSUB >= 1; RSUB >>= 1) consider(kTD[tdi], kTH[thi], RSUB, NSUB, kLdsBudget);
  };
  search();
  if (!have && (xlead >= 0 || dvec)) { xlead = -1; dvec = 0; search(); }
  if (!have) return CRN_EINVAL;
  if (xlead < 0) dvec = 0;
  if (xlead < 0 || !dvec) {
    WgCand c;
    if (!wg_cand(best.TD, best.TH, best.TW, best.RSUB, best.NSUB, x->C, Npad, kd, kh, kw, xlead, dvec, 150 * 1024, &c)) {
      have = false; search();
      if (!have) return CRN_EINVAL;
    } else {
      best = c;
    }
  }
  WgradGeom g{};
  g.x = *x; g.dy = *dy;
  if (tr) g.tr = *tr; else g.tr = crnInTransform{nullptr, nullptr, 0, 0};
  g.dw = dw; g.Npad = Npad;
  g.lead = xlead >= 0 ? xlead : 0;
  g.kd = kd; g.kh = kh; g.kw = kw; g.pd = pd; g.ph = ph; g.pw = pw + g.lead; g.T = T;
  g.TD = best.TD; g.TH = best.TH; g.TW = best.TW;
  g.PD = g.TD + kd - 1; g.PH = g.TH + kh - 1; g.PW = best.PW;
  g.PSP = best.PSP; g.POSP = best.POSP;
  const int NSUB = best.NSUB, RSUB = best.RSUB, NB = NSUB * 16, CC = best.CC;
  const int npos = g.TD * g.TH * g.TW;
  g.CC = CC;
  g.tilesD = crn_cdiv(Dy, g.TD); g.tilesH = crn_cdiv(Hy, g.TH); g.tilesW = crn_cdiv(Wy, g.TW);
  g.ntiles = g.tilesD * g.tilesH * g.tilesW * dy->B;
  const int cblocks = crn_cdiv(x->C, CC), nblocks = crn_cdiv(Npad, NB);
  constexpr int budget = 512;
  int splits = std::max(1, std::min(g.ntiles, budget / (cblocks * nblocks)));
  if (crn_deterministic()) splits = 1;
  g.tiles_per_split = crn_cdiv(g.ntiles, splits);
  splits = crn_cdiv(g.ntiles, g.tiles_per_split);
  bool balanced = false;
  if (boxes && boxes->n_groups > 0 && boxes->n_groups <= 8 && dy->C % boxes->n_groups == 0 &&
      (dy->C / boxes->n_groups) % NB == 0) {
    balanced = true;
    g.n_groups = boxes->n_groups; memcpy(g.n_box, boxes->n_box, sizeof(g.n_box));
    double w[8], wsum = 0.0;
    for (int gi = 0; gi < g.n_groups; ++gi) {
      const signed char* b = boxes->n_box[gi];
      w[gi] = 0.35 * T + std::max(0, b[1] - b[0]) * std::max(0, b[3] - b[2]) * std::max(0, b[5] - b[4]);
      wsum += w[gi];
    }
    g.balanced = 1; g.nbpg = (dy->C / boxes->n_groups) / NB;
    g.zoff[0] = 0;
    for (int gi = 0; gi < g.n_groups; ++gi) {
      const int sgi = crn_deterministic() ? 1 : std::max(1, std::min(g.ntiles, (int)(splits * w[gi] * g.n_groups / wsum + 0.5)));
      g.tps[gi] = crn_cdiv(g.ntiles, sgi);
      g.sg[gi] = crn_cdiv(g.ntiles, g.tps[gi]);
      g.zoff[gi + 1] = g.zoff[gi] + g.nbpg * g.sg[gi];
    }
  }
  g.lg2 = ilog2_ceil(g.PH * g.PW); g.npass = xlead >= 0 ? 0 : stage_passes(CC * g.PD, g.PH * g.PW);
  g.dlg2 = ilog2_ceil(npos); g.dnpass = dvec ? 0 : stage_passes(NB, npos);
  g.magic_PW = magic20(g.PW); g.magic_PD = magic20(g.PD); g.magic_T = magic20(T);
  g.magic_TW = magic20(g.TW); g.magic_TH = magic20(g.TH);
  if (xlead >= 0) {
    g.plu = g.PH * g.PW / 4; g.pw4 = g.PW / 4; g.nunits = CC * g.PD * g.plu;
    g.magic_PLU = magic20(g.plu); g.magic_PW4 = magic20(g.pw4);
  }
  if (dvec) { g.np4 = npos / (dvec == 2 ? 2 : 4); g.dnunits = NB * g.np4; g.magic_NP4 = magic20(g.np4); }
  g.Tfull = T; g.khf = kh; g.kwf = kw; g.ncols = Npad; g.xcd = 1;
  dim3 grid((unsigned)cblocks, (unsigned)(g.balanced ? 1 : nblocks), (unsigned)(g.balanced ? g.zoff[g.n_groups] : splits));
  const size_t lds_bytes = best.lds;
#define CRN_WG_CASE(R, N) \
  if (RSUB == R && NSUB == N) return crn_launch_wgrad_##R##_##N(g, xlead >= 0, dvec, grid, lds_bytes, st);
  CRN_WG_CONFIGS(CRN_WG_CASE)
#undef CRN_WG_CASE
  return CRN_EINVAL;
}
}

extern "C" int crn_conv_wgrad(const crnView* x, const crnInTransform* tr, const crnView* dy,
                              float* dw, int Npad, int kd, int kh, int kw, int pd, int ph, int pw,
                              int zero_first, const crnTapBoxes* boxes, crnStream stream) {
  CRN_ENTRY(stream);
  if (!x || !dy || !dw || Npad <= 0 || (Npad & 15) || x->B != dy->B) return CRN_EINVAL;
  hipStream_t st = (hipStream_t)stream;
  const int T = kd * kh * kw;
  if (T > 512) return CRN_EINVAL;
  if (zero_first) CRN_HIP(hipMemsetAsync(dw, 0, (size_t)x->C * T * Npad * 4, st));
  if (T == 1 && one_position(*x) && one_position(*dy) && dy->C >= 1024) {
    const crnInTransform trv = tr ? *tr : crnInTransform{nullptr, nullptr, 0, 0};
    hipLaunchKernelGGL(dense_wgrad_kernel, dim3((unsigned)crn_cdiv(dy->C, 256), (unsigned)x->C), dim3(256), 0, st, x->base,
                       x->sB, x->sC, trv, dy->base, dy->sB, dy->sC, dw, Npad, dy->C, x->C, x->B);
    CRN_CHECK_LAUNCH();
    return CRN_OK;
  }
  return wgrad_launch(x, tr, dy, dw, Npad, kd, kh, kw, pd, ph, pw, boxes, st);
}
```

corenet_amd/csrc/misc_ops.hip:

```cpp
#include "crn_common.h"
#include <cstdlib>
#include <algorithm>
#include <cmath>

namespace {

__global__ void preprocess_kernel(const uint8_t* img, int64_t HW, float* out, int64_t total) {
  const int64_t e = blockIdx.x * (int64_t)blockDim.x + threadIdx.x;
  if (e >= total) return;
  const int64_t s = e % HW;
  const int c = (int)((e / HW) % 3);
  const int64_t b = e / (3 * HW);
  const float mean = c == 0 ? 103.939f : (c == 1 ? 116.779f : 123.68f);
  out[e] = (float)img[(b * 3 + (2 - c)) * HW + s] + mean;
}

__global__ void bn_relu_maxpool_fwd_kernel(const float* x, const float* scale, const float* shift,
                                           int C, int H, int W, int Ho, int Wo, float* y,
                                           int32_t* argmax, int64_t total) {
  const int64_t e = blockIdx.x * (int64_t)blockDim.x + threadIdx.x;
  if (e >= total) return;
  const int ow = (int)(e % Wo);
  const int oh = (int)((e / Wo) % Ho);
  const int64_t bc = e / ((int64_t)Wo * Ho);
// ... 371 lines not shown
  }
  if (dw) {
    hipLaunchKernelGGL(linear_bwd_dw_kernel, dim3(nblk((int64_t)N * K)), dim3(256), 0, (hipStream_t)s, x, dy, lddy, B,
                       K, N, dw, db);
    CRN_CHECK_LAUNCH();
  }
  return CRN_OK;
}

extern "C" int crn_fill_offset_channels(float* x, int B, int64_t sB, int64_t S, int c0, const float* offset,
                                        crnStream s) {
  CRN_ENTRY(s);
  const int64_t total = (int64_t)B * 3 * S;
  hipLaunchKernelGGL(fill_offset_kernel, dim3(nblk(total)), dim3(256), 0, (hipStream_t)s, x, sB, S, c0, offset, total);
  CRN_CHECK_LAUNCH();
  return CRN_OK;
}

extern "C" int crn_decoder_inputs(const float* v2s, const float* offset, int B, int nscales, const float* scales, float* layer_mats,
                                  float* offset_out, crnStream s) {
  CRN_ENTRY(s);
  if (!v2s || !offset || !scales || !layer_mats || !offset_out || B < 1 || nscales < 1 || nscales > 4) return CRN_EINVAL;
  float f[4] = {1.f, 1.f, 1.f, 1.f};
  for (int i = 0; i < nscales; ++i) f[i] = scales[i];
  hipLaunchKernelGGL(decoder_inputs_kernel, dim3(nblk((int64_t)nscales * B * 16)), dim3(256), 0, (hipStream_t)s, v2s, offset, B, nscales,
                     f[0], f[1], f[2], f[3], layer_mats, offset_out);
  CRN_CHECK_LAUNCH();
  return CRN_OK;
}

extern "C" int crn_gather_f32(const float* src, const int32_t* idx, float* dst, int64_t n, crnStream s) {
  CRN_ENTRY(s);
  hipLaunchKernelGGL(gather_kernel, dim3(std::min(nblk(n), 4096u)), dim3(256), 0, (hipStream_t)s, src, idx, dst, n);
  CRN_CHECK_LAUNCH();
  return CRN_OK;
}

extern "C" int crn_scatter_f32(const float* src, const int32_t* idx, float* dst, int64_t n, int accumulate,
                               crnStream s) {
  CRN_ENTRY(s);
  hipLaunchKernelGGL(scatter_kernel, dim3(std::min(nblk(n), 4096u)), dim3(256), 0, (hipStream_t)s, src, idx, dst, n,
                     accumulate);
  CRN_CHECK_LAUNCH();
  return CRN_OK;
}

extern "C" int crn_copy_tiles_f32(const float* src, float* dst, const int32_t* desc, const uint64_t* mask,
                                  const int32_t* explicit_idx, int64_t ntiles, int reverse, crnStream s) {
  CRN_ENTRY(s);
  if (!src || !dst || !desc || !mask || ntiles < 0) return CRN_EINVAL;
  if (ntiles == 0) return CRN_OK;
  constexpr int64_t kCap = 16384;
  const unsigned blocks = (unsigned)std::min<int64_t>(crn_cdiv(ntiles, 4), kCap);
  if (reverse)
    hipLaunchKernelGGL(copy_tiles_kernel<true>, dim3(blocks), dim3(256), 0, (hipStream_t)s, src, dst, desc,
                       reinterpret_cast<const unsigned long long*>(mask), explicit_idx, ntiles);
  else
    hipLaunchKernelGGL(copy_tiles_kernel<false>, dim3(blocks), dim3(256), 0, (hipStream_t)s, src, dst, desc,
                       reinterpret_cast<const unsigned long long*>(mask), explicit_idx, ntiles);
  CRN_CHECK_LAUNCH();
  return CRN_OK;
}

extern "C" int crn_copy_mats_f32(const float* src, float* dst, const int32_t* desc, int64_t ntiles, int reverse, crnStream s) {
  CRN_ENTRY(s);
  if (!src || !dst || !desc || ntiles < 0) return CRN_EINVAL;
  if (ntiles == 0) return CRN_OK;
  constexpr int64_t kCap = 8192;
  const unsigned blocks = (unsigned)std::min<int64_t>(ntiles, kCap);
  if (reverse)
    hipLaunchKernelGGL(copy_mats_kernel<true>, dim3(blocks), dim3(256), 0, (hipStream_t)s, src, dst, desc, ntiles);
  else
    hipLaunchKernelGGL(copy_mats_kernel<false>, dim3(blocks), dim3(256), 0, (hipStream_t)s, src, dst, desc, ntiles);
  CRN_CHECK_LAUNCH();
  return CRN_OK;
}

extern "C" int crn_zero_f32(float* p, int64_t n, crnStream s) {
  CRN_ENTRY(s);
  CRN_HIP(hipMemsetAsync(p, 0, (size_t)n * 4, (hipStream_t)s));
  return CRN_OK;
}

extern "C" int crn_add_i64(int64_t* p, int n, int64_t v, crnStream s) {
  CRN_ENTRY(s);
  hipLaunchKernelGGL(add_i64_kernel, dim3(nblk(n)), dim3(256), 0, (hipStream_t)s, p, n, v);
  CRN_CHECK_LAUNCH();
  return CRN_OK;
}

extern "C" int crn_adam_step(float* param, const float* grad, float* exp_avg, float* exp_avg_sq, int64_t n,
                             float lr, float beta1, float beta2, float eps, float grad_scale, int step,
                             crnStream s) {
  CRN_ENTRY(s);
  if (step < 1 || n < 1) return CRN_EINVAL;
  if (((uintptr_t)param | (uintptr_t)grad | (uintptr_t)exp_avg | (uintptr_t)exp_avg_sq) & 15) return CRN_EINVAL;
  const double bc1 = 1.0 - std::pow((double)beta1, step), bc2 = 1.0 - std::pow((double)beta2, step);
  const int64_t n4 = n / 4;
  hipLaunchKernelGGL(adam_kernel, dim3(std::min(nblk(n4), 8192u)), dim3(256), 0, (hipStream_t)s, param, grad, exp_avg,
                     exp_avg_sq, n4, n, lr, beta1, beta2, eps, grad_scale, (float)bc1, (float)std::sqrt(bc2));
  CRN_CHECK_LAUNCH();
  return CRN_OK;
}

extern "C" int crn_adam_set_hyper(float* hyper, float lr, float beta1, float beta2, float eps, float grad_scale,
                                  int step, crnStream s) {
  CRN_ENTRY(s);
  if (!hyper || step < 1) return CRN_EINVAL;
  const double bc1 = 1.0 - std::pow((double)beta1, step), bc2 = 1.0 - std::pow((double)beta2, step);
  hipLaunchKernelGGL(set_hyper_kernel, dim3(1), dim3(64), 0, (hipStream_t)s, hyper, lr, beta1, beta2, eps, grad_scale,
                     (float)bc1, (float)std::sqrt(bc2));
  CRN_CHECK_LAUNCH();
  return CRN_OK;
}

extern "C" int crn_adam_step_hyper(float* param, const float* grad, float* exp_avg, float* exp_avg_sq, int64_t n,
                                   const float* hyper, crnStream s) {
  CRN_ENTRY(s);
  if (n < 1 || !hyper) return CRN_EINVAL;
  if (((uintptr_t)param | (uintptr_t)grad | (uintptr_t)exp_avg | (uintptr_t)exp_avg_sq) & 15) return CRN_EINVAL;
  const int64_t n4 = n / 4;
  hipLaunchKernelGGL(adam_hyper_kernel, dim3(std::min(nblk(n4), 8192u)), dim3(256), 0, (hipStream_t)s, param, grad,
                     exp_avg, exp_avg_sq, n4, n, hyper);
  CRN_CHECK_LAUNCH();
  return CRN_OK;
}

namespace {
__global__ __launch_bounds__(256) void stride2_gather_kernel(const float* __restrict__ x, float* __restrict__ y,
                                                             int h, int w, int64_t planes) {
  const int64_t t = blockIdx.x * (int64_t)blockDim.x + threadIdx.x;
  const int w2 = w >> 1;
  const int64_t n = planes * h * w2;
  if (t >= n) return;
  const int j2 = (int)(t % w2);
  const int64_t r = t / w2;
  const int i = (int)(r % h);
  const int64_t p = r / h;
  const f32x4 v = *reinterpret_cast<const f32x4*>(x + (p * (2 * h) + 2 * i) * (int64_t)(2 * w) + 4 * j2);
  typedef float f32x2 __attribute__((ext_vector_type(2)));
  *reinterpret_cast<f32x2*>(y + (p * h + i) * (int64_t)w + 2 * j2) = (f32x2){v[0], v[2]};
}
__global__ __launch_bounds__(256) void stride2_scatter_kernel(const float* __restrict__ dy, float* __restrict__ dx,
                                                              int h, int w, int64_t planes) {
  const int64_t t = blockIdx.x * (int64_t)blockDim.x + threadIdx.x;
  const int w2 = w >> 1;
  const int64_t n = planes * (2 * h) * w2;
  if (t >= n) return;
  const int j2 = (int)(t % w2);
  const int64_t r = t / w2;
  const int io = (int)(r % (2 * h));
  const int64_t p = r / (2 * h);
  f32x4 v = (f32x4){0.f, 0.f, 0.f, 0.f};
  if ((io & 1) == 0) {
    const float* s = dy + (p * h + (io >> 1)) * (int64_t)w + 2 * j2;
    v[0] = s[0]; v[2] = s[1];
  }
  *reinterpret_cast<f32x4*>(dx + (p * (2 * h) + io) * (int64_t)(2 * w) + 4 * j2) = v;
}
__global__ __launch_bounds__(256) void stride2_gather_any_kernel(const float* __restrict__ x, float* __restrict__ y, int h, int w,
                                                                 int hin, int win, int64_t planes) {
  const int64_t t = blockIdx.x * (int64_t)blockDim.x + threadIdx.x;
  if (t >= planes * h * w) return;
  const int j = (int)(t % w);
  const int64_t r = t / w;
  const int i = (int)(r % h);
// ... 52 lines not shown
```

corenet_amd/model/engine.py:

```python
from __future__ import annotations

import dataclasses
import os
from typing import Dict, List, Optional, Tuple

import numpy as np
import torch as t

from corenet_amd import _lib
from corenet_amd import views as V
from corenet_amd.backend import Transform
from corenet_amd.model import conv_geometry as G

IMAGE_HW = (256, 256)


def check_image_hw(hw):
  H, W = int(hw[0]), int(hw[1])
  if H < 32 or W < 32 or H % 4 or W % 4 or H * W > 4096 * 4096:
    raise ValueError(f"corenet_amd.CoreNet: image batch of {H}x{W} pixels; this engine takes H and W that are multiples of 4 and >= 32 "
                     f"(256x256 in every shipped config)")
  return H, W
BN_EPS = 1e-3
BN_MOMENTUM = 0.01
# ... 47 lines not shown
  for st in range(2, 7):
    cmid, cout, k1, k2 = chans[st]
    p = f"{d}stage_{st}."
    bn(p + "b1.", cin)
    conv(p + "c1.", cmid, cin, k1, k1, k1)
    bn(p + "b2.", cmid)
    specs.append((p + "t1.weight", (cmid, cout, k2, k2, k2), "param"))
    specs.append((p + "t1.bias", (cout,), "param"))
    if st in src_c:
      sk = round(cout * skip_fraction)
      conv(f"{d}rt_skip_{st}.compress_channels.", sk, src_c[st] + 3, 1, 1)
      cin = cout + sk
  return specs


class ParamStore:

  def __init__(self, specs, device, dtype=t.float32):
    self.specs = specs
    self.device = device
    self.off: Dict[str, Tuple[int, Tuple[int, ...]]] = {}
    np_, nb, nn = 0, 0, 0
    for key, shape, kind in specs:
      n = int(np.prod(shape)) if len(shape) else 1
      n4 = (n + 3) // 4 * 4
      if kind == "param":
        self.off[key] = (np_, shape); np_ += n4
      elif kind == "buffer":
        self.off[key] = (nb, shape); nb += n4
      else:
        self.off[key] = (nn, shape); nn += 1
    self.kind = {k: kd for k, _, kd in specs}
    self.params = t.zeros(np_, dtype=dtype, device=device)
    self.gslab = t.zeros(np_ + nb, dtype=dtype, device=device)
    self.grads = self.gslab[:np_]
    self.buf_stage = self.gslab[np_:]
    self.buffers = t.zeros(nb, dtype=dtype, device=device)
    self.nbt = t.zeros(nn, dtype=t.int64, device=device)

  def slab(self, key):
    return {"param": self.params, "buffer": self.buffers, "nbt": self.nbt}[self.kind[key]]

  def view(self, key, grad=False) -> t.Tensor:
    o, shape = self.off[key]
    n = int(np.prod(shape)) if len(shape) else 1
    slab = self.grads if grad else self.slab(key)
    return slab[o:o + n].view(shape)

  def offset(self, key) -> int:
    return self.off[key][0]

  def view_of(self, slab: t.Tensor, key) -> t.Tensor:
    o, shape = self.off[key]
    n = int(np.prod(shape)) if len(shape) else 1
    return slab[o:o + n].view(shape)


@dataclasses.dataclass
class BN:
  C: int
  gamma: t.Tensor
  beta: t.Tensor
  rmean: t.Tensor
  rvar: t.Tensor
  nbt: t.Tensor
  dgamma: t.Tensor
  dbeta: t.Tensor
  scale: t.Tensor
  shift: t.Tensor
  saved: t.Tensor


@dataclasses.dataclass
class Conv:
  name: str
  fwd: G.Geom
  dgrad: Optional[G.Geom]
  wf: t.Tensor
  wd: Optional[t.Tensor]
  bias: t.Tensor
  gwf: t.Tensor
  dbias: t.Tensor
  n_ref: int
  wop_f: Optional[t.Tensor] = None
  wop_d: Optional[t.Tensor] = None
  wop_kind: str = ""
  ct_f: Optional[t.Tensor] = None
  ct_d: Optional[t.Tensor] = None
  ct_kind: str = ""


@dataclasses.dataclass(slots=True, eq=False)
class EncBlock:
  prefix: str; stage: str; cin: int; f: Tuple[int, int, int]; stride: int; h: int; w: int
  down: bool
  final: bool
  ya: t.Tensor; yb: t.Tensor; yc: t.Tensor; ys: Optional[t.Tensor]; out: t.Tensor
  gpre: t.Tensor; gyc: t.Tensor; gab: t.Tensor; gyb: t.Tensor; gaa: t.Tensor; gya: t.Tensor
  gys: Optional[t.Tensor]; gin: Optional[t.Tensor]
  xs: Optional[t.Tensor]; gxs: Optional[t.Tensor]
  xs_next: Optional["EncBlock"] = None
  inp: Optional[t.Tensor] = None
  xs_filled: bool = False


@dataclasses.dataclass(slots=True, eq=False)
class DecStage:
  cin: int; cmid: int; cout: int; r: int
  u: t.Tensor; gu: t.Tensor; w: t.Tensor; gw: t.Tensor; gv1: t.Tensor; gv2: t.Tensor

  def __getitem__(self, field: str):
    return getattr(self, field)


class on_stream:
  __slots__ = ("stream", "after", "_torch", "_pin")

  def __init__(self, stream, after=None):
    self.stream, self.after = stream, after
    self._torch, self._pin = t.cuda.stream(stream), _lib.pinned_stream(stream)

  def __enter__(self):
    self._torch.__enter__(); self._pin.__enter__()
    if self.after is not None:
      self.stream.wait_event(self.after)

  def __exit__(self, *exc):
    self._pin.__exit__(*exc); self._torch.__exit__(*exc)


_NO_KW = {}
_ORPHANS = []


class Engine:

  def __init__(self, num_classes: int, resolution=(128, 128, 128), latent_channels: int = 64,
               skip_fraction: float = 0.75, last_upscale_factor: int = 2, device="cuda",
               backend=None, dtype=t.float32, decoder_math: Optional[str] = None):
    if tuple(resolution) != (128, 128, 128) or last_upscale_factor != 2:
      raise ValueError("the CoReNet decoder is only defined for resolution 128^3, "
                       "last_upscale_factor 2 (reconstruction_decoder.py:38-54,93-95)")
    if backend is None:
      from corenet_amd.backend import default_backend
      backend = default_backend()
    self.be = backend
    default_math = "bf16x3" if getattr(backend, "name", "") == "hip" else "fp32"
    self.decoder_math = decoder_math or os.environ.get("CRN_DECODER_MATH", default_math)
    if self.decoder_math not in ("fp32", "bf16x3"):
      raise ValueError(f"decoder_math must be 'fp32' or 'bf16x3', not {self.decoder_math!r}")
    self.encoder_e2d = self.decoder_math == "bf16x3"
    assert dtype == t.float32 or getattr(backend, "name", "") == "emu"
    self.dtype = dtype
    self.device = t.device(device)
    if self.device.type == "cuda" and self.device.index is None:
      self.device = t.device("cuda", t.cuda.current_device() if t.cuda.is_available() else 0)
    self.num_classes = num_classes
    self.latent = latent_channels
    self.resolution = tuple(resolution)
    self.specs = param_specs(num_classes, latent_channels, skip_fraction)
    self.store = ParamStore(self.specs, self.device, dtype)
    self.skip_ch = {2: round(128 * skip_fraction), 3: round(64 * skip_fraction),
                    4: round(32 * skip_fraction), 5: round(16 * skip_fraction)}
    self._build_layers()
    self.plans: Dict[int, "Plan"] = {}
    self.adam_m: Optional[t.Tensor] = None
# ... 40 lines not shown

  def release_graph_resources(self):
    for p in self.plans.values():
      for g in list(p.graphs.values()) + ([p.eval_graph] if p.eval_graph is not None else []):
        try:
          g.reset()
        except Exception:
          pass
      p.graphs, p.eval_graph, p.eval_eager = {}, None, 0
    if self._capture is not None:
      self.be.splitk_release(self._capture)
      self._capture = None

  def side_stream(self):
    if self._side is False:
      use = self.device.type == "cuda"
      self._side = t.cuda.Stream(device=self.device) if use else None
      if use:
        self._pack_ev, self._dgrad_packed = t.cuda.Event(), t.cuda.Event()
        self._dec_packed, self._enc_late_packed = t.cuda.Event(), t.cuda.Event()
    return self._side

  def _bn(self, prefix: str) -> BN:
    s = self.store
    c = s.off[prefix + "weight"][1][0]
    dev = self.device
    o = self._bn_slab_off[prefix]
    return BN(c, s.view(prefix + "weight"), s.view(prefix + "bias"), s.view(prefix + "running_mean"),
              s.view(prefix + "running_var"), s.view(prefix + "num_batches_tracked"),
              s.view(prefix + "weight", grad=True), s.view(prefix + "bias", grad=True),
              self.bn_scale[o:o + c], self.bn_shift[o:o + c],
              t.zeros(4 * c, device=dev, dtype=self.dtype))

  def _bn_slabs(self):
    s = self.store
    self._bn_slab_off, rows, n = {}, [], 0
    for key, shape, kind in self.specs:
      if not key.endswith("running_mean"):
        continue
      p = key[:-len("running_mean")]
      c = shape[0]
      self._bn_slab_off[p] = n
      ch = np.arange(c)
      rows.append(np.stack([s.offset(p + "weight") + ch, s.offset(p + "bias") + ch, s.offset(p + "running_mean") + ch,
                            s.offset(p + "running_var") + ch, n + ch], 1))
      n += (c + 3) // 4 * 4
    self.bn_scale = t.zeros(n, device=self.device, dtype=self.dtype)
    self.bn_shift = t.zeros(n, device=self.device, dtype=self.dtype)
    self.bn_eval_table = t.as_tensor(np.concatenate(rows).astype(np.int32), device=self.device)

  def bn_eval_affine(self):
    self.be.bn_eval_affine(self.store.params, self.store.buffers, self.bn_eval_table, BN_EPS, self.bn_scale,
                           self.bn_shift)

  def _build_layers(self):
    s = self.store
    self.convs: Dict[str, Conv] = {}
    self.bns: Dict[str, BN] = {}
    self._bn_slabs()
    reg: List[Tuple[str, G.Geom, Optional[G.Geom], int, int]] = []

    def add(name, fwd, dgrad, repeat=1):
      nref = s.off[name + "bias"][1][0]
      reg.append((name, fwd, dgrad, repeat, nref))

    for key, shape, kind in self.specs:
      if kind != "param" or not key.endswith("weight") or len(shape) < 4:
        if key.endswith("running_mean"):
          p = key[:-len("running_mean")]
          self.bns[p] = self._bn(p)
        continue
      name = key[:-len("weight")]
      if name == "encoder.stage1.conv.":
        add(name, G.stem_fwd(shape, 3), None)
      elif name == "decoder.stage_1.t1.":
        add(name, G.convt_1to4_fwd(shape), G.convt_1to4_dgrad(shape), repeat=64)
      elif ".t1." in name:
        p = 1 if shape[2] == 3 else 3
        add(name, G.convt_fwd(shape, p), G.convt_dgrad(shape, p), repeat=8)
      else:
        p = shape[-1] // 2
        add(name, G.conv_fwd(shape, p), G.conv_dgrad(shape, p))
    idx_parts, sizes = [], []
    for name, fwd, dgrad, repeat, nref in reg:
      wo, bo = s.offset(name + "weight"), s.offset(name + "bias")
      def shift(ix, o):
        return np.where(ix >= 0, ix.astype(np.int64) + o, -1)
      parts = [shift(fwd.index, wo), shift(G.bias_index(nref, repeat, fwd.npad, parity_major=(repeat == 8)), bo)]
      if dgrad is not None:
        alias = (len(dgrad.index) == int(np.prod(s.off[name + "weight"][1]))
                 and np.array_equal(dgrad.index, np.arange(len(dgrad.index))))
        parts.append(np.zeros(0, np.int64) if alias else shift(dgrad.index, wo))
      idx_parts.append(parts)
    flat_len = sum(len(p) for parts in idx_parts for p in parts)
    assert max(int(p.max()) for parts in idx_parts for p in parts if len(p)) < 2 ** 31
    self.packed = t.zeros(flat_len, dtype=self.dtype, device=self.device)
    gsize = sum(len(parts[0]) for parts in idx_parts)
    self.gpacked = t.zeros(gsize, dtype=self.dtype, device=self.device)
    pack_parts, pack_is_bwd, pack_names, unpack_parts = [], [], [], []
    po, go = 0, 0
    for (name, fwd, dgrad, repeat, nref), parts in zip(reg, idx_parts):
      pack_parts.append((po, parts[0], fwd.npad, 0)); po += len(parts[0]); pack_is_bwd.append(False); pack_names.append(name)
      pack_parts.append((po, parts[1], len(parts[1]), 0)); po += len(parts[1]); pack_is_bwd.append(False); pack_names.append(name)
      if dgrad is not None and len(parts[2]):
        pack_parts.append((po, parts[2], dgrad.npad, dgrad.taps if dgrad.taps > 1 else 0)); po += len(parts[2])
        pack_is_bwd.append(True); pack_names.append(name)
      unpack_parts.append((go, parts[0], fwd.npad, 0)); go += len(parts[0])
    dev = self._tiles_dev
    self.pack_tiles = dev([pp for pp, bwd in zip(pack_parts, pack_is_bwd) if not bwd])
    sel = lambda pred: [pp for pp, bwd, nm in zip(pack_parts, pack_is_bwd, pack_names) if not bwd and pred(nm)]
    early = lambda nm: nm.startswith("encoder.stage1") or nm.startswith("encoder.stage2")
    self.pack_tiles_enc = dev(sel(lambda nm: nm.startswith("encoder.")))
    self.pack_tiles_enc_early = dev(sel(early))
    self.pack_tiles_enc_late = dev(sel(lambda nm: nm.startswith("encoder.") and not early(nm)))
    self.pack_tiles_dec = dev(sel(lambda nm: not nm.startswith("encoder.")))
    self.pack_tiles_bwd = dev([pp for pp, bwd in zip(pack_parts, pack_is_bwd) if bwd])
    self.unpack_tiles = dev(unpack_parts)
    los = [min(o for k, (o, _) in s.off.items() if s.kind[k] == "param" and k.startswith(lb))
           for lb in GRAD_BUCKET_LABELS[:-1]] + [0]
    self.grad_buckets: List[Tuple[str, int, int]] = []
    self._bucket_tiles = []
    hi = s.params.numel()
    for lb, lo in zip(GRAD_BUCKET_LABELS, los):
      assert lo < hi
      self.grad_buckets.append((lb, lo, hi))
      sel = [up for (name, *_), up in zip(reg, unpack_parts) if lo <= s.offset(name + "weight") < hi]
      self._bucket_tiles.append(sel)
      hi = lo
    self._bucket_dev = None
    po, go = 0, 0
    for (name, fwd, dgrad, repeat, nref), parts in zip(reg, idx_parts):
      nwf, nb = len(parts[0]), len(parts[1])
      wf = self.packed[po:po + nwf]; po += nwf
      bias = self.packed[po:po + nb]; po += nb
      wd = None
      if dgrad is not None:
        if len(parts[2]):
          wd = self.packed[po:po + len(parts[2])]; po += len(parts[2])
        else:
          wd = s.view(name + "weight").view(-1)
      gwf = self.gpacked[go:go + nwf]; go += nwf
      self.convs[name] = Conv(name, fwd, dgrad, wf, wd, bias, gwf,
                              s.view(name + "bias", grad=True), nref)
    self._build_operands(reg, idx_parts)

  def _build_ct_images(self):
    self.ct_tables = {}
    name = "decoder.stage_6.t1."
    if (self.decoder_math != "bf16x3" or self.device.type != "cuda"
        or name not in self.convs or not hasattr(self.be, "convt_par_fwd")):
      return
    shape = tuple(self.store.off[name + "weight"][1])
    if shape[0] != 16 or shape[1] > 16 or tuple(shape[2:]) != (7, 7, 7) or tuple(self.resolution) != (128, 128, 128):
      return
    if shape[1] == 2:
      kind_, tabs = "res", (G.convt_res_fwd_table, G.convt_res_dgrad_table)
    elif shape[1] >= CT_PAR_MIN:
      kind_, tabs = "par", (G.convt_par_fwd_table, G.convt_par_dgrad_table)
    else:
      return
    self.convs[name].ct_kind = kind_
    wofs = self.store.offset(name + "weight")
    for kind, fn, field in (("dec", tabs[0], "ct_f"), ("bwd", tabs[1], "ct_d")):
      tab, nbytes = fn(shape, wofs)
      img = t.zeros(nbytes, dtype=t.uint8, device=self.device)
      setattr(self.convs[name], field, img)
      self.ct_tables[kind] = (t.as_tensor(tab, device=self.device), img)

  def _build_operands(self, reg, idx_parts):
    self.wop = None
    self.op_tables = {}
    self._build_ct_images()
    if self.decoder_math != "bf16x3":
      return
    groups = {"enc_early": [], "enc_late": [], "dec": [], "bwd": []}
    slices = []
    po, eo = 0, 0
    for (name, fwd, dgrad, repeat, nref), parts in zip(reg, idx_parts):
      src_f = po; po += len(parts[0]) + len(parts[1])
      src_d = po
      if dgrad is not None:
        po += len(parts[2])
      if (name, "fwd") in BF16X3_LAUNCHES:
        groups["dec"].append((src_f, eo, fwd, True))
        slices.append((name, "wop_f", eo, G.slab_entries(fwd))); eo += G.slab_entries(fwd)
        groups["bwd"].append((src_d, eo, dgrad, True))
        slices.append((name, "wop_d", eo, G.slab_entries(dgrad))); eo += G.slab_entries(dgrad)
        self.convs[name].wop_kind = "slab"
        continue
      if not self.encoder_e2d or not name.startswith("encoder.") or name.startswith("encoder.stage1"):
        continue
      self.convs[name].wop_kind = "e2d"
      if fwd.window != (1, 3, 3):
        continue
      if G.operand_eligible(fwd) and name[len("encoder.stage")] in "45":
        groups["enc_early" if name.startswith("encoder.stage2") else "enc_late"].append((src_f, eo, fwd))
        slices.append((name, "wop_f", eo, G.operand_entries(fwd))); eo += G.operand_entries(fwd)
      if dgrad is not None and len(parts[2]) and G.operand_eligible(dgrad):
        groups["bwd"].append((src_d, eo, dgrad))
        slices.append((name, "wop_d", eo, G.operand_entries(dgrad))); eo += G.operand_entries(dgrad)
    if not eo:
      return
    self.wop = t.zeros(eo * 32, dtype=t.uint8, device=self.device)
    for name, field, e0, n in slices:
      setattr(self.convs[name], field, self.wop[e0 * 32:(e0 + n) * 32])
    for k, layers in groups.items():
      if layers:
        desc, blocks = G.operand_table(layers)
        self.op_tables[k] = (t.as_tensor(desc, device=self.device), blocks)

  def _operands(self, *groups):
    for k in groups:
      if k in self.op_tables:
        self.be.bf3_operands(self.packed, self.op_tables[k], self.wop)
      if k in self.ct_tables:
        self.be.bf3_gather_image(self.store.params, *self.ct_tables[k])

  def _tiles_dev(self, parts):
    mats, rest = G.mat_index(parts)
    tl = G.tile_index(rest)
    return (t.as_tensor(tl[0], device=self.device), t.as_tensor(tl[1].view(np.int64), device=self.device),
            t.as_tensor(tl[2] if tl[2].size else np.zeros(1, np.int32), device=self.device),
            t.as_tensor(mats, device=self.device))

  def bucket_unpack_tiles(self, i: int):
    if self._bucket_dev is None:
      self._bucket_dev = [self._tiles_dev(sel) for sel in self._bucket_tiles]
    return self._bucket_dev[i]

  @property
  def weights_dirty(self) -> bool:
    return self._weights_dirty

  @weights_dirty.setter
  def weights_dirty(self, v: bool):
    self._weights_dirty = v
    if v:
      self.dgrad_dirty = True

  def pack_weights(self, part: str = "all"):
    tiles = {"all": self.pack_tiles, "enc": self.pack_tiles_enc, "dec": self.pack_tiles_dec,
             "enc_early": self.pack_tiles_enc_early, "enc_late": self.pack_tiles_enc_late}[part]
    self.be.copy_tiles(self.store.params, self.packed, tiles)
    self._operands(*{"all": ("enc_early", "enc_late", "dec"), "enc": ("enc_early", "enc_late"), "dec": ("dec",),
                     "enc_early": ("enc_early",), "enc_late": ("enc_late",)}[part])
    if part in ("all", "dec"):
      self._weights_dirty = False

  def pack_dgrad_weights(self):
    self.be.copy_tiles(self.store.params, self.packed, self.pack_tiles_bwd)
    self._operands("bwd")
    self.dgrad_dirty = False

  def plan(self, batch: int, hw=IMAGE_HW) -> "Plan":
    hw = (int(hw[0]), int(hw[1]))
    key = batch if hw == IMAGE_HW else (batch, hw[0], hw[1])
    p = self.plans.get(key)
    if p is None:
      p = Plan(self, batch, hw)
      self.plans[key] = p
    return p

  def adam_step(self, lr: float, eps: float, betas=(0.9, 0.999), grad_scale: float = 1.0):
    if self.adam_m is None:
      self.adam_m = t.zeros_like(self.store.params)
      self.adam_v = t.zeros_like(self.store.params)
    self.adam_t += 1
    self.be.adam_step(self.store.params, self.store.grads, self.adam_m, self.adam_v,
                      self.store.params.numel(), lr, betas[0], betas[1], eps, grad_scale, self.adam_t)
    self.weights_dirty = True

  def adam_step_graphable(self, lr: float, eps: float, betas=(0.9, 0.999), grad_scale: float = 1.0, launch: bool = True):
    if self.adam_m is None:
      self.adam_m = t.zeros_like(self.store.params)
      self.adam_v = t.zeros_like(self.store.params)
    if self.adam_hyper is None:
      self.adam_hyper = t.zeros(8, dtype=t.float32, device=self.device)
    self.adam_t += 1
    self.be.adam_set_hyper(self.adam_hyper, lr, betas[0], betas[1], eps, grad_scale, self.adam_t)
    if launch:
      self.adam_update_from_hyper()

  def adam_bucket_hook(self):
    def hook(gslice: t.Tensor):
      lo, n = gslice.storage_offset(), gslice.numel()
      self.be.adam_step_hyper(self.store.params[lo:lo + n], gslice, self.adam_m[lo:lo + n], self.adam_v[lo:lo + n], n,
                              self.adam_hyper)
    return hook

  def adam_update_from_hyper(self):
    self.be.adam_step_hyper(self.store.params, self.store.grads, self.adam_m, self.adam_v,
                            self.store.params.numel(), self.adam_hyper)
    self.weights_dirty = True


def _no_exchange(grads: t.Tensor):
  """Bucket hook of a step without a gradient exchange."""


class Plan:

  def __init__(self, eng: Engine, B: int, hw=IMAGE_HW):
    self.eng, self.B = eng, B
    H, W = check_image_hw(hw)
    self.hw = (H, W)
    self.stem_hw = (H // 2, W // 2)
# ... 105 lines not shown

  probes = None

  def _probe(self, name: str, fn):
    if self.probes is None or name not in self.probes:
      return fn()
    a, b = t.cuda.Event(enable_timing=True), t.cuda.Event(enable_timing=True)
    a.record(); r = fn(); b.record()
    self.probes[name].append((a, b))
    return r

  @property
  def overlap(self) -> bool:
    return self.side is not None and self.trace is None

  def _on_side(self, after=None):
    return on_stream(self.side, after)

  def _next_handover_event(self):
    if self._side_i == len(self._side_ev):
      self._side_ev.append(t.cuda.Event())
    ev = self._side_ev[self._side_i]; self._side_i += 1
    ev.record()
    return ev

  def _stats(self, bn: BN, x: t.Tensor, S: int, sB: int, pre_relu: bool, training: bool):
    if not training:
      return
    with _lib.roctx_range("bn_stats C%d S%d" % (bn.C, S)):
      self.be.bn_stats(x, self.B, bn.C, S, sB, pre_relu, bn.gamma, bn.beta, bn.rmean, bn.rvar, bn.nbt,
                       BN_EPS, BN_MOMENTUM, True, bn.scale, bn.shift, bn.saved)

  def _bn_finalize(self, b: BN, parts: int, count: int):
    self.be.bn_finalize(parts, b.C, count, b.gamma, b.beta, b.rmean, b.rvar, b.nbt, BN_EPS, BN_MOMENTUM, b.scale, b.shift, b.saved)

  def _bn_bwd(self, b: BN, x: t.Tensor, dy: t.Tensor, dx: t.Tensor, S: int, pre_relu: bool, post_relu: bool, bias_of: Optional[Conv] = None):
    n = b.C * S
    self.be.bn_bwd(x, n, dy, n, self.B, b.C, S, pre_relu, post_relu, b.gamma, b.scale, b.shift, b.saved, dx, n, b.dgamma, b.dbeta,
                   dsum=None if bias_of is None else bias_of.dbias, ndsum=0 if bias_of is None else bias_of.n_ref)

  trace = None

  def _timed(self, label, fn):
    if _lib.ROCTX:
      with _lib.roctx_range(label):
        return fn()
    if self.trace is None:
      return fn()
    a, b = t.cuda.Event(enable_timing=True), t.cuda.Event(enable_timing=True)
    a.record(); r = fn(); b.record()
    self.trace.append((label, a, b))
    return r

  def _math(self, cv: Conv, direction: str) -> str:
    if cv.wop_kind == "e2d" and (direction == "fwd" and cv.wop_f is not None or
                                 direction == "dgrad" and cv.wop_d is not None):
      return "e2d"
    return "bf16x3" if self.eng.decoder_math == "bf16x3" and (cv.name, direction) in BF16X3_LAUNCHES else "fp32"

  conv_positions = None

  @staticmethod
  def _e2d_shape_ok(v: V.View, window) -> bool:
    S = v.D * v.H * v.W
    if S % 4:
      return False
    if tuple(window) == (1, 3, 3):
      tw = 16 if v.W % 16 == 0 else 8
      return v.D == 1 and v.W % tw == 0 and v.H % (64 // tw) == 0
    return S % 64 == 0

  @staticmethod
  def _wg2d_shape_ok(v: V.View, window) -> bool:
    return (v.D * v.H * v.W) % 32 == 0 and (tuple(window) == (1, 1, 1) or v.W % 8 == 0)

  def _conv(self, cv: Conv, x: V.View, tr, y: V.View, accumulate=False):
    g = cv.fwd
    if self.conv_positions is not None:
      self.conv_positions[cv.name] = y.D * y.H * y.W
    if cv.wop_f is not None and cv.wop_kind == "e2d" and self._e2d_shape_ok(y, g.window):
      self._timed("fwd   " + cv.name, lambda: self.be.conv2d_bf3(
          x, tr, cv.wop_f, g.npad, cv.bias, 0, y, g.window, g.pad_lo, accumulate))
      return
    self._timed("fwd   " + cv.name, lambda: self.be.conv_fwd(
        x, tr, cv.wf, g.npad, cv.bias, 0, y, g.window, g.pad_lo, 0, accumulate, boxes=(g.n_boxes, g.c_boxes),
        math=self._math(cv, "fwd"), wslab=cv.wop_f if cv.wop_kind == "slab" else None))

  def _dgrad(self, cv: Conv, dy: V.View, dx: V.View, accumulate=False):
    g = cv.dgrad
    if cv.wop_d is not None and cv.wop_kind == "e2d" and self._e2d_shape_ok(dx, g.window):
      self._timed("dgrad " + cv.name, lambda: self.be.conv2d_bf3(
          dy, None, cv.wop_d, g.npad, None, 0, dx, g.window, g.pad_lo, accumulate))
      return
    self._timed("dgrad " + cv.name, lambda: self.be.conv_fwd(
        dy, None, cv.wd, g.npad, None, 0, dx, g.window, g.pad_lo, 0, accumulate, boxes=(g.n_boxes, g.c_boxes),
        math=self._math(cv, "dgrad"), wslab=cv.wop_d if cv.wop_kind == "slab" else None))

  def _dgrad_bn_bwd(self, cv: Conv, dy: V.View, g: t.Tensor, x: t.Tensor, Cn: int, S: int, b, dx: t.Tensor, cprev: Conv) -> bool:
    be = self.be
    gvw = self.vw(g)
    fusable = (hasattr(be, "conv_dgrad_bn_bwd") and cv.wop_kind == "slab" and cv.wop_d is not None
               and self._math(cv, "dgrad") == "bf16x3")
    if not fusable:
      be.splitk_defer()
      self._dgrad(cv, dy, gvw)
      return False
    gd = cv.dgrad
    be.splitk_defer()
    return self._timed("dgrad " + cv.name, lambda: be.conv_dgrad_bn_bwd(
        dy, cv.wop_d, gd.npad, gvw, g, gd.window, gd.pad_lo, (gd.n_boxes, gd.c_boxes), x, Cn * S, self.B, Cn, S, True, b.gamma,
        b.scale, b.shift, b.saved, dx, Cn * S, b.dgamma, b.dbeta, dsum=cprev.dbias, ndsum=cprev.n_ref))

  def _wgrad_math(self, cv: Conv, dy: V.View) -> str:
    g = cv.fwd
    math = self._math(cv, "wgrad")
    if self.stem_fast and cv.name == "encoder.stage1.conv.":
      math = "stem"
    if (self.eng.encoder_e2d and g.window in ((1, 1, 1), (1, 3, 3)) and self._wg2d_shape_ok(dy, g.window)
        and (cv.name.startswith("encoder.stage") and not cv.name.startswith("encoder.stage1")
             or cv.name.startswith("decoder.rt_skip"))):
      math = "bf16x3_2d"
    if cv.ct_kind == "par" and math == "bf16x3":
      math = "ct_par"
    return math

  def _launch_wgrad(self, cv: Conv, x: V.View, tr, dy: V.View, math: str, kw: dict):
    g = cv.fwd
    with _lib.roctx_range("wgrad " + cv.name):
      self.be.conv_wgrad(x, tr, dy, cv.gwf, g.npad, g.window, g.pad_lo, False, boxes=(g.n_boxes, g.c_boxes), math=math, **kw)

  def _wgrad(self, cv: Conv, x: V.View, tr, dy: V.View, here: bool = False):
    math = self._wgrad_math(cv, dy)
    kw = self._ximg_kw(math)
    if here:
      return self._launch_wgrad(cv, x, tr, dy, math, kw)
    if not self.overlap:
      return self._timed("wgrad " + cv.name, lambda: self._launch_wgrad(cv, x, tr, dy, math, kw))
    if cv.name.startswith("encoder."):
      self._wg_pending.append((cv, x, tr, dy, math, kw))
      return
    if self._handed_over:
      self._handed_over = False
      self._side_i = max(self._side_i, 1)
      ev = None
    else:
      ev = self._next_handover_event()
    with self._on_side(after=ev):
      self._launch_wgrad(cv, x, tr, dy, math, kw)

  def _ximg_kw(self, math: str) -> dict:
    if math != "ct_par" or self._ct_ximg is None:
      return _NO_KW
    img, self._ct_ximg = self._ct_ximg, None
    return {"ximg": img}

  def _flush_wgrads(self, then=None):
    if not self._wg_pending and then is None:
      return
    with self._on_side(after=self._next_handover_event()):
      for args in self._wg_pending:
        self._launch_wgrad(*args)
      if then is not None:
        then()
    self._wg_pending = []

  def _join_side(self):
    self._flush_wgrads()
    if self._side_i:
      self._side_done.record(self.side)
      t.cuda.current_stream().wait_event(self._side_done)
      self._side_i = 0

  def _bias_grad(self, cv: Conv, dy: t.Tensor, S: int, sB: int):
    self.be.bias_grad(dy, self.B, cv.n_ref, S, sB, cv.dbias)

  def forward(self, image_u8: t.Tensor, v2s: t.Tensor, offset: t.Tensor, training: bool) -> t.Tensor:
    self._skip_async_live = bool(training and self.overlap)
    if self._skip_async_live:
      self._decoder_inputs(v2s, offset)
    self.forward_encoder(image_u8, training)
    try:
      return self.forward_decoder(v2s, offset, training)
    finally:
      self._skip_async_live = False

  def _decoder_inputs(self, v2s: t.Tensor, offset: t.Tensor):
    B = self.B
    if (hasattr(self.be, "decoder_inputs") and v2s.dtype == self.layer_mats.dtype and offset.dtype == self.offset.dtype
        and v2s.is_contiguous() and offset.is_contiguous() and v2s.device == self.layer_mats.device):
      self.be.decoder_inputs(v2s, offset, self._layer_scale_list, self.layer_mats, self.offset)
      return
    self.offset.copy_(offset)
    v = v2s.to(self.layer_mats.dtype).reshape(1, B, 4, 4)
    self.layer_mats.copy_((v * self.layer_scales).reshape(4, B, 16))

  def _skip_fwd(self, k: int):
    eng, be, B = self.eng, self.be, self.B
    d = self.dec[k]
    out = self.dec[k + 1].u
    ft = self.feat[self.skip_src[k]]
    (hh, ww), ro = self.skip_hw[k], 2 * d.r
    be.fill_offset_channels(ft, B, ft.stride(0), ft.shape[2] * ft.shape[3], ft.shape[1] - 3, self.offset)
    self._conv(eng.convs[f"decoder.rt_skip_{k}.compress_channels."], self.vw(ft), None,
               self.vw(self.smap[k].permute(0, 3, 1, 2)))
    if self.ray_idx is not None and self.training:
      self._probe(f"ray_sample_fwd_{ro}", lambda: be.ray_sample_fwd_idx(
          self.smap[k], self.smap[k].stride(0), B, eng.skip_ch[k], hh, ww, self.layer_mats[k - 2],
          self.offset, out[:, d.cout:], out.stride(0), ro, ro, ro, self.ray_idx[k], map_sC=1, map_sP=eng.skip_ch[k]))
    else:
      self._probe(f"ray_sample_fwd_{ro}", lambda: be.ray_sample_fwd(
          self.smap[k], self.smap[k].stride(0), B, eng.skip_ch[k], hh, ww, self.layer_mats[k - 2],
# ... 132 lines not shown
    p = blk.prefix
    S = blk.h * blk.w
    f1, f2, f3 = blk.f
    if blk.stride == 2:
      if blk.xs_filled:
        blk.xs_filled = False
      else:
        be.stride2_gather(cur, blk.xs)
      xin = self.vw(blk.xs)
    else:
      xin = self.vw(cur)
    ba, bb, bc = bn[p + "op_a.bn."], bn[p + "op_b.bn."], bn[p + "op_c.bn."]
    defer = be.splitk_defer if training else (lambda: None)
    defer()
    self._conv(cv[p + "op_a.conv."], xin, None, self.vw(blk.ya))
    self._stats(ba, blk.ya, S, f1 * S, False, training)
    defer()
    self._conv(cv[p + "op_b.conv."], self.vw(blk.ya), Transform(ba.scale, ba.shift, post_relu=True), self.vw(blk.yb))
    self._stats(bb, blk.yb, S, f2 * S, False, training)
    if blk.final:
      pre, sB_pre = self.feat[blk.stage], self.feat[blk.stage].stride(0)
    else:
      pre, sB_pre = None, 0
    fused_tail = training and hasattr(be, "bn_stats_tail")
    res, rsc, rsh = cur, None, None
    def shortcut():
      bs = bn[p + "shortcut.bn."]
      defer()
      self._conv(cv[p + "shortcut.conv."], xin, None, self.vw(blk.ys))
      self._stats(bs, blk.ys, S, f3 * S, False, training)
      return blk.ys, bs.scale, bs.shift
    if blk.down and fused_tail:
      res, rsc, rsh = shortcut()
    defer()
    self._conv(cv[p + "op_c.conv."], self.vw(blk.yb), Transform(bb.scale, bb.shift, post_relu=True), self.vw(blk.yc))
    if fused_tail:
      nxt = blk.xs_next
      with _lib.roctx_range("bn_stats_tail C%d S%d" % (bc.C, S)):
        be.bn_stats_tail(blk.yc, B, f3, S, f3 * S, bc.gamma, bc.beta, bc.rmean, bc.rvar, bc.nbt, BN_EPS, BN_MOMENTUM,
                         True, bc.scale, bc.shift, bc.saved, res, rsc, rsh, f3 * S, pre, sB_pre, blk.out, f3 * S, True,
                         y2=nxt.xs if nxt is not None else None, W=blk.w)
      if nxt is not None:
        nxt.xs_filled = True
    else:
      self._stats(bc, blk.yc, S, f3 * S, False, training)
      if blk.down:
        res, rsc, rsh = shortcut()
      be.affine_add_relu(blk.yc, bc.scale, bc.shift, res, rsc, rsh, B, f3, S, f3 * S, f3 * S, pre, sB_pre, blk.out, f3 * S, True)
    blk.inp = cur
    return blk.out

  def _grads_ready(self, label: str, hook):
    if hook is None:
      self._flush_wgrads()
      return
    eng = self.eng
    i = [b[0] for b in eng.grad_buckets].index(label)
    _, lo, hi = eng.grad_buckets[i]
    tiles = eng.bucket_unpack_tiles(i)
    def run():
      if tiles[0].numel() or tiles[3].numel():
        self.be.copy_tiles(eng.gpacked, eng.store.grads, tiles, reverse=True)
      hook(eng.store.grads[lo:hi])
    if not self.overlap:
      return run()
    return self._flush_wgrads(then=run)

  def backward(self, glogits: t.Tensor, grad_hook=None):
    eng, be, B = self.eng, self.be, self.B
    cv, bn = eng.convs, eng.bns
    assert self.training, "backward needs a training-mode forward"
    if eng._dgrad_pack_pending:
      t.cuda.current_stream().wait_event(eng._dgrad_packed)
      eng._dgrad_pack_pending = False
    elif eng.dgrad_dirty:
      eng.pack_dgrad_weights()
    if not eng._gpacked_zeroed:
      be.zero(eng.gpacked)
    eng._gpacked_zeroed = False
    overlap = self.overlap
    if overlap:
      with self._on_side():
        be.zero(self.gsmap_slab)
      if grad_hook is None:
        grad_hook = _no_exchange
    else:
      be.zero(self.gsmap_slab)
    L = eng.latent
    g_out = glogits
    for k in range(6, 1, -1):
      d = self.dec[k]
      S, So = d.r ** 3, (2 * d.r) ** 3
      p = f"decoder.stage_{k}."
      b1_, b2_ = bn[p + "b1."], bn[p + "b2."]
      ctot = g_out.shape[1]
      if k < 6:
        if overlap:
          self._skip_bwd_ev[k].record()
          with self._on_side(after=self._skip_bwd_ev[k]):
            self._skip_bwd(k, g_out, on_side=True)
            if k == 2:
              self._skip_bwd_done.record(self.side)
          self._handed_over = True
        else:
          self._skip_bwd(k, g_out, on_side=False)
      ct = cv[p + "t1."]
      gv = self.s2d(g_out, d.cout, (2, 2, 2))
      tr2 = Transform(b2_.scale, b2_.shift, pre_relu=True)
      self._wgrad(ct, self.vw(d.w), tr2, gv)
      self._handed_over = False
      if k == 6:
        if overlap:
          with self._on_side():
            self._bias_grad(ct, g_out, So, ctot * So)
        else:
          self._bias_grad(ct, g_out, So, ctot * So)
      cc = cv[p + "c1."]
      if ct.ct_d is not None and self._math(ct, "dgrad") == "bf16x3":
        self._timed("dgrad " + ct.name, lambda: be.convt_par_dgrad(g_out, d.cout, ct.ct_d, d.gv2, False, resident=ct.ct_kind == "res"))
        ct_done = False
      else:
        ct_done = self._dgrad_bn_bwd(ct, gv, d.gv2, d.w, d.cmid, S, b2_, d.gw, cc)
      if not ct_done:
        self._bn_bwd(b2_, d.w, d.gv2, d.gw, S, True, False, bias_of=cc)
      tr1 = Transform(b1_.scale, b1_.shift, pre_relu=True)
      self._wgrad(cc, self.vw(d.u), tr1, self.vw(d.gw))
      cprev = cv[f"decoder.stage_{k - 1}.t1."]
      if not self._dgrad_bn_bwd(cc, self.vw(d.gw), d.gv1, d.u, d.cin, S, b1_, d.gu, cprev):
        self._bn_bwd(b1_, d.u, d.gv1, d.gu, S, True, False, bias_of=cprev)
      g_out = d.gu
      if k == 3:
        self._grads_ready("decoder.stage_3.", grad_hook)
    c1 = cv["decoder.stage_1.t1."]
    b = bn["decoder.stage_1.b1."]
    zv = self.vw(self.z0.view(B, L + 3, 1, 1, 1))
    gv = self.flat(g_out)
    self._wgrad(c1, zv, Transform(b.scale, b.shift, pre_relu=True), gv)
    self._dgrad(c1, gv, self.vw(self.gv0.view(B, L + 3, 1, 1, 1)))
    self._bn_bwd(b, self.z0, self.gv0, self.gz0, 1, True, False)
    s = eng.store
    be.linear_bwd(self.avg, s.view("decoder.stage_0.weight"), self.gz0, L + 3, B, 2048, L, self.gavg,
                  s.view("decoder.stage_0.weight", grad=True), s.view("decoder.stage_0.bias", grad=True))
    self._grads_ready("decoder.stage_0.", grad_hook)
    if overlap:
      t.cuda.current_stream().wait_event(self._skip_bwd_done)
    f5, g5 = self.feat["stage5"], self.gfeat["stage5"]
    last = self.blocks[-1]
    S5 = f5.shape[2] * f5.shape[3]
    be.relu_mean_bwd(f5, self.gavg, B, 2048, S5, f5.stride(0), last.gpre, 2048 * S5, False)
    be.affine_add_relu(last.gpre, None, None, g5, None, None, B, 2048, S5, 2048 * S5, g5.stride(0),
                       None, 0, last.gpre, 2048 * S5, False)
    g_in = None
    for blk in reversed(self.blocks):
      g_in = self._block_bwd(blk, g_in)
      self._flush_wgrads()
      if blk.prefix in GRAD_BUCKET_LABELS:
        self._grads_ready(blk.prefix, grad_hook)
    b1 = bn["encoder.stage1_part2.bn."]
    H1, W1 = self.stem_hw
    be.maxpool_bwd(g_in, self.p1_arg, B, 64, H1, W1, self.gy1)
    cs = cv["encoder.stage1.conv."]
    self._bn_bwd(b1, self.y1, self.gy1, self.gy1b, H1 * W1, False, False, bias_of=cs)
    self._wgrad(cs, self.s2d(self.img, 3, (1, 2, 2)), None, self.vw(self.gy1b))
    self._grads_ready("", grad_hook)
    self._join_side()
    if grad_hook is None:
      be.copy_tiles(eng.gpacked, eng.store.grads, eng.unpack_tiles, reverse=True)

  def _ray_bwd(self, k: int, g_out: t.Tensor):
    d, gm = self.dec[k], self.gsmap[k]
# ... 73 lines not shown
```

include/corenet_hip.h:

```cpp
#ifndef CORENET_HIP_H_
#define CORENET_HIP_H_

#include <stddef.h>
#include <stdint.h>

#ifdef __cplusplus
extern "C" {
#endif

#define CRN_OK 0
#define CRN_EINVAL (-1)
#define CRN_ENOMEM (-2)
#define CRN_ENOCONV (-3)

typedef void* crnStream;

typedef struct {
  float* base;
  int32_t B, C, D, H, W;
  int64_t sB, sC;
  const int32_t* chan_off;
  int32_t sD, sH, sW;
} crnView;

typedef struct {
  const float* scale;
  const float* shift;
  int32_t pre_relu, post_relu;
} crnInTransform;

typedef struct {
  int32_t n_groups, c_groups;
  int8_t n_box[8][6];
  int8_t c_box[8][6];
} crnTapBoxes;

int crn_conv_fwd(const crnView* x, const crnInTransform* tr, const float* w, int Npad,
                 const float* bias, int bias_sB, const crnView* y,
                 int kd, int kh, int kw, int pd, int ph, int pw,
                 int splits, int accumulate ,
                 const crnTapBoxes* boxes , crnStream stream);

int crn_conv_fwd_bf3(const crnView* x, const crnInTransform* tr, const float* w, int Npad,
                     const float* bias, int bias_sB, const crnView* y,
                     int kd, int kh, int kw, int pd, int ph, int pw,
                     int accumulate, const crnTapBoxes* boxes , crnStream stream);

int crn_conv_fwd_bf3_slabs(const crnView* x, const crnInTransform* tr, const void* wslab, int Npad,
                           const float* bias, int bias_sB, const crnView* y,
                           int kd, int kh, int kw, int pd, int ph, int pw,
                           int accumulate, const crnTapBoxes* boxes , crnStream stream);

typedef struct crnBnBwdFuse {
  const float* x;
  int64_t sB_x;
  const float* saved;
  int pre_relu;
  double* ws; size_t ws_bytes;
  float* dsum; int ndsum;
  int nparts;
} crnBnBwdFuse;
int crn_conv_fwd_bf3_slabs_bnbwd(const crnView* x, const crnInTransform* tr, const void* wslab, int Npad,
                                 const float* bias, int bias_sB, const crnView* y,
                                 int kd, int kh, int kw, int pd, int ph, int pw,
                                 int accumulate, const crnTapBoxes* boxes , crnBnBwdFuse* fuse,
                                 crnStream stream);

int crn_conv_fwd_bf3_slabs_stats(const crnView* x, const crnInTransform* tr, const void* wslab, int Npad,
                                 const float* bias, int bias_sB, const crnView* y,
                                 int kd, int kh, int kw, int pd, int ph, int pw,
                                 int accumulate, const crnTapBoxes* boxes , int pre_relu,
                                 double* ws, size_t ws_bytes, int* nparts, crnStream stream);

int crn_splitk_defer(int on);
int crn_splitk_reserve(int64_t floats, crnStream stream);
int crn_splitk_release(crnStream stream);

int crn_conv_wgrad(const crnView* x, const crnInTransform* tr, const crnView* dy,
                   float* dw, int Npad, int kd, int kh, int kw, int pd, int ph, int pw,
                   int zero_first, const crnTapBoxes* boxes ,
                   crnStream stream);

int crn_conv_wgrad_bf3(const crnView* x, const crnInTransform* tr, const crnView* dy,
                       float* dw, int Npad, int kd, int kh, int kw, int pd, int ph, int pw,
                       int zero_first, crnStream stream);
int crn_conv_wgrad_bf3_boxes(const crnView* x, const crnInTransform* tr, const crnView* dy, float* dw, int Npad,
                             int kd, int kh, int kw, int pd, int ph, int pw, int zero_first,
                             const crnTapBoxes* boxes , crnStream stream);

int crn_bf3_operands(const float* packed, const int64_t* desc, int nlayers, int64_t total_blocks, void* out,
                     crnStream stream);
int crn_conv2d_bf3(const crnView* x, const crnInTransform* tr, const void* wop, int Npad, const float* bias,
                   int bias_sB, const crnView* y, int kh, int kw, int ph, int pw, int accumulate, crnStream stream);

int crn_conv_wgrad_1x1_bf3(const crnView* x, const crnInTransform* tr, const crnView* dy, float* dw, int Npad,
                           int zero_first, crnStream stream);
int crn_conv_wgrad_2d_bf3(const crnView* x, const crnInTransform* tr, const crnView* dy, float* dw, int Npad,
                          int kh, int kw, int ph, int pw, int zero_first, crnStream stream);

int crn_copy_tiles_f32(const float* src, float* dst, const int32_t* desc ,
                       const uint64_t* mask , const int32_t* explicit_idx, int64_t ntiles,
                       int reverse, crnStream s);
int crn_copy_mats_f32(const float* src, float* dst, const int32_t* desc , int64_t nblocks,
                      int reverse, crnStream s);
int crn_gather_f32(const float* src, const int32_t* idx, float* dst, int64_t n, crnStream s);
int crn_scatter_f32(const float* src, const int32_t* idx, float* dst, int64_t n,
                    int accumulate, crnStream s);
int crn_bias_grad(const float* dy, int B, int C, int64_t S, int64_t sB, float* db,
                  int accumulate, double* workspace ,
                  size_t workspace_bytes, crnStream s);

int crn_batch_renorm_stats(const float* x, int B, int C, int64_t S, int64_t sB, int pre_relu,
                           const float* gamma, const float* beta,
                           float* running_mean, float* running_var,
                           const int64_t* num_batches_tracked ,
                           float eps, float momentum, int training,
                           float* scale, float* shift, float* saved ,
                           double* workspace, size_t workspace_bytes, crnStream s);
size_t crn_batch_renorm_workspace_bytes(int C);
int crn_batch_renorm_stats_tail(const float* x, int B, int C, int64_t S, int64_t sB,
                                const float* gamma, const float* beta, float* running_mean, float* running_var,
                                const int64_t* num_batches_tracked, float eps, float momentum, int training,
                                float* scale, float* shift, float* saved, double* workspace, size_t workspace_bytes,
                                const float* r, const float* rscale, const float* rshift, int64_t sB_r,
                                float* y_pre, int64_t sB_pre, float* y, int64_t sB_y, int relu,
                                float* y2, int W, crnStream s);

int crn_batch_renorm_eval_affine(const float* params, const float* buffers, const int32_t* table,
                                 int n, float eps, float* scale, float* shift, crnStream s);

int crn_batch_renorm_bwd(const float* x, int64_t sB_x, const float* dy, int64_t sB_dy,
                         int B, int C, int64_t S, int pre_relu, int post_relu,
                         const float* gamma, const float* scale, const float* shift,
                         const float* saved, float* dx, int64_t sB_dx,
                         float* dgamma, float* dbeta, int accumulate,
                         float* dsum, int ndsum,
                         double* workspace, size_t workspace_bytes, crnStream s);

int crn_batch_renorm_bwd_apply(const float* x, int64_t sB_x, const float* dy, int64_t sB_dy,
                               int B, int C, int64_t S, int pre_relu,
                               const float* gamma, const float* scale, const float* shift,
                               const float* saved, float* dx, int64_t sB_dx,
                               float* dgamma, float* dbeta, int accumulate,
                               float* dsum, int ndsum,
                               double* workspace, size_t workspace_bytes, int nparts, crnStream s);

int crn_batch_renorm_bwd_head(const float* x, int64_t sB_x, float* dy, int64_t sB_dy,
                              const float* g, int64_t sB_g, const float* act, int64_t sB_act,
                              const float* g2 , int64_t sB_g2,
                              int B, int C, int64_t S, const float* gamma, const float* scale, const float* shift,
                              const float* saved, float* dx, int64_t sB_dx, float* dgamma, float* dbeta,
                              int accumulate, float* dsum, int ndsum,
                              double* workspace, size_t workspace_bytes, const float* g_compact, int W, crnStream s);

int crn_affine_add_relu(const float* x, const float* scale, const float* shift,
                        const float* r, const float* rscale, const float* rshift,
                        int B, int C, int64_t S, int64_t sB_x, int64_t sB_r,
                        float* y_pre, int64_t sB_pre, float* y, int64_t sB_y,
                        int relu, crnStream s);

int crn_relu_bwd_add(const float* dy, const float* y_pre, const float* dy2,
                     int B, int C, int64_t S, int64_t sB_dy, int64_t sB_pre, int64_t sB_dy2,
                     float* dx, int64_t sB_dx, crnStream s);

size_t crn_stem_conv_parts(int B, int H, int W);
int crn_stem_conv_fwd(const float* img, int B, int H, int W, const float* w_packed, const float* bias,
                      float* y, double* stats_ws , size_t ws_bytes, crnStream s);
int crn_stem_conv_wgrad(const float* img, int B, int H, int W, const float* dy, float* dw_packed, crnStream s);
int crn_batch_renorm_finalize(const double* ws, int nparts, int C, double count,
                              const float* gamma, const float* beta, float* running_mean, float* running_var,
                              const int64_t* nbt, float eps, float momentum,
                              float* scale, float* shift, float* saved, crnStream s);

int crn_preprocess_caffe(const uint8_t* img, int B, int H, int W, float* out, crnStream s);
int crn_bn_relu_maxpool_fwd(const float* x, const float* scale, const float* shift,
                            int B, int C, int H, int W, float* y, int32_t* argmax, crnStream s);
int crn_bn_relu_maxpool_bwd(const float* dy, const int32_t* argmax, int B, int C, int H, int W,
                            float* dx_bn , crnStream s);
int crn_relu_mean_fwd(const float* x_pre, int B, int C, int64_t S, int64_t sB, float* avg, crnStream s);
// ... 53 lines not shown
                             const void* wimg, float* dx, int64_t dx_sB, int accumulate, crnStream s);
int crn_convt_s2k7_c2_fwd_bf3(const float* x, int64_t x_sB, int B, int D, int H, int W, const crnInTransform* tr,
                              const void* wimg, const float* bias, float* y, int64_t y_sB, int64_t y_sC, int Cout, crnStream s);
int crn_convt_s2k7_c2_dgrad_bf3(const float* dy, int64_t dy_sB, int64_t dy_sC, int Cout, int B, int D, int H, int W,
                                const void* wimg, float* dx, int64_t dx_sB, int accumulate, crnStream s);
int crn_convt_s2k7_wgrad_bf3(const float* x, int64_t x_sB, int B, int D, int H, int W, const crnInTransform* tr,
                             const float* dy, int64_t dy_sB, int64_t dy_sC, int Cout, float* dw, int Npad, int zero_first,
                             const void* ximg, crnStream s);
size_t crn_convt_s2k7_ximage_bytes(int B, int D, int H, int W);
int crn_convt_s2k7_ximage(const float* x, int64_t x_sB, int B, int D, int H, int W, const crnInTransform* tr,
                          void* img, size_t img_bytes, crnStream s);

int crn_fill_voxels(const void* grid, void* out, int dtype, int N, int D, int H, int W,
                    void* workspace, size_t workspace_bytes, crnStream s);
size_t crn_fill_voxels_workspace_bytes(int N, int D, int H, int W);
int crn_fill_voxels_strided(const void* grid, const int64_t* grid_strides, void* out, const int64_t* out_strides,
                            int dtype, int N, int D, int H, int W, void* workspace, size_t workspace_bytes, crnStream s);

int crn_fill_voxels_cpu(const void* grid, void* out, int dtype, int N, int D, int H, int W,
                        int num_threads);

#define CRN_MC_MAX_OBJECT_CELLS ((int64_t)1 << 29)
size_t crn_marching_cubes_workspace_bytes(int N, int D, int H, int W);
int crn_marching_cubes_count(const float* grid, const int64_t* strides, int N, int D, int H, int W, float level,
                             void* workspace, size_t workspace_bytes, int64_t* counts, crnStream s);
int crn_marching_cubes_emit(const float* grid, const int64_t* strides, int N, int D, int H, int W, float level,
                            const float* matrices, void* workspace, size_t workspace_bytes, float* vertices,
                            float* normals, int32_t* faces, crnStream s);
int crn_box_filter(const float* in, const int64_t* strides, float* out, int N, int D, int H, int W, int k,
                   void* workspace, size_t workspace_bytes, crnStream s);
int crn_marching_cubes_cpu(const float* grid, const int64_t* strides, int N, int D, int H, int W, float level,
                           const float* matrices, int64_t* counts, float* vertices, float* normals, int32_t* faces,
                           int num_threads);
int crn_box_filter_cpu(const float* in, const int64_t* strides, float* out, int N, int D, int H, int W, int k,
                       int num_threads);

#define CRN_RENDER_TILE 16
typedef struct {
  float vp[16];
  float light[3], cam[3], light_color[3], ambient_light[3], clear[3];
  int32_t cull, normal_mode, t0, t1, inst0, pad[4];
} crnRenderImage;
int crn_render_bin(const float* triangles, const crnRenderImage* images, int I, int H, int W, int max_len,
                   int64_t num_inst, float* records, int32_t* bin_counts, int64_t* bin_offsets, crnStream s);
int crn_render_raster(const float* triangles, const float* normals, const int32_t* material_ids, const float* materials,
                      int M, const crnRenderImage* images, int I, int H, int W, int max_len, const float* records,
                      int32_t* bin_counts, const int64_t* bin_offsets, int32_t* bin_list, uint8_t* out, crnStream s);
int crn_render_cpu(const float* triangles, const float* normals, const int32_t* material_ids, const float* materials,
                   int M, const crnRenderImage* images, int I, int H, int W, uint8_t* out, int num_threads);
size_t crn_voxel_faces_workspace_bytes(int N, int D, int H, int W);
int crn_voxel_faces_count(const int32_t* labels, int N, int D, int H, int W, const float* palette, int P,
                          const float* box_matrices, float* box_out, void* workspace, size_t workspace_bytes,
                          int64_t* counts, crnStream s);
int crn_voxel_faces_emit(const int32_t* labels, int N, int D, int H, int W, const float* palette, int P,
                         const float* matrices, int material_base, void* workspace, size_t workspace_bytes,
                         float* triangles, float* normals, int32_t* material_ids, crnStream s);
int crn_voxel_faces_cpu(const int32_t* labels, int N, int D, int H, int W, const float* palette, int P,
                        const float* box_matrices, float* box_out, const float* matrices, int material_base,
                        int64_t* counts, float* triangles, float* normals, int32_t* material_ids, int num_threads);

int crn_voxelize_mesh(const float* triangles, const int32_t* tri_mesh, int T,
                      const float* view2voxel, int M, int D, int H, int W,
                      int sub_grid_side, float image_resolution_multiplier,
                      int conservative, int depth_multiplier, float* grid, crnStream s);
int crn_transform_meshes(const float* triangles, const int32_t* tri_mesh, int T,
                         const float* mesh_matrix, int M, float* out, crnStream s);
int crn_merge_labels(const float* meshes_grid, const int32_t* scene_mesh_start,
                     const int32_t* mesh_label, int B, int D, int H, int W, int sub_grid,
                     int32_t* out, crnStream s);

int crn_comm_unique_id(void* id128 );
int crn_comm_init(const void* id128, int rank, int nranks, void** comm);
int crn_comm_destroy(void* comm);
int crn_comm_info(void* comm , int* rccl_version, int* rank, int* nranks);
int crn_allreduce_f32(void* comm, float* buf, int64_t n, crnStream s);
int crn_broadcast_f32(void* comm, float* buf, int64_t n, int root, crnStream s);

int crn_roctx_push(const char* label);
int crn_roctx_pop(void);

int crn_set_deterministic(int on);

int crn_zero_f32(float* p, int64_t n, crnStream s);
int crn_add_i64(int64_t* p, int n, int64_t v, crnStream s);
const char* crn_version(void);

#ifdef CRN_TOOLS
int crn_bf3_debug_stamps(long long* out192);
int crn_e2d_debug_stamps(long long* out32);
int crn_pw_debug_stamps(long long* out32);
#endif

#ifdef __cplusplus
}
#endif
#endif
```

Baseline: 1.190 billion.

## Read and write pointwise conv weights directly in native N-by-C slab layout

Adds pointwise forward and 1x1 wgrad kernel variants that read weights and write gradients in the parameter store's native [N][C] layout. For eligible encoder 1x1 convs this removes the weight pack copy and the gradient unpack copy. The wgrad variant reduces partial sums across waves in shared memory, then atomically adds into the gradient slab, so slab gradient ranges must be zeroed up front by a new range-zero kernel. The added cost is transposed shared-memory staging, extra atomics, and a fallback path that copies tiles into scratch buffers.

```diff
diff --git a/corenet_amd/_lib.py b/corenet_amd/_lib.py
--- a/corenet_amd/_lib.py
+++ b/corenet_amd/_lib.py
@@ -148,6 +148,9 @@
     "crn_transform_meshes": [vp, vp, i32, vp, i32, vp, vp],
     "crn_merge_labels": [vp, vp, vp, i32, i32, i32, i32, i32, vp, vp],
     "crn_zero_f32": [vp, i64, vp],
+    "crn_zero_ranges_f32": [vp, vp, i64, vp],
+    "crn_conv_fwd_pointwise_nc": [C.POINTER(CrnView), C.POINTER(CrnInTransform), vp, vp, i32, C.POINTER(CrnView), i32, i32, vp],
+    "crn_conv_wgrad_1x1_bf3_nc": [C.POINTER(CrnView), C.POINTER(CrnInTransform), C.POINTER(CrnView), vp, i32, vp],
     "crn_add_i64": [vp, i32, i64, vp],
 }
 _SIZE_FNS = {
diff --git a/corenet_amd/backend.py b/corenet_amd/backend.py
--- a/corenet_amd/backend.py
+++ b/corenet_amd/backend.py
@@ -90,6 +90,21 @@
                           C.byref(_cview(y)), window[0], window[1], window[2],
                           pad_lo[0], pad_lo[1], pad_lo[2], splits, int(accumulate), _ctapboxes(boxes),
                           _lib.stream())
+
+  def conv_fwd_pointwise_nc(self, x: View, tr: Optional[Transform], w: t.Tensor, bias: Optional[t.Tensor], bias_sB: int,
+                            y: View, accumulate: bool = False) -> bool:
+    rc = self.lib._crn_conv_fwd_pointwise_nc(C.byref(_cview(x)), _ctr(tr), ptr(w), ptr(bias), bias_sB, C.byref(_cview(y)),
+                                             0, int(accumulate), _lib.stream())
+    if rc not in (0, -1):
+      raise _lib.HipError(f"crn_conv_fwd_pointwise_nc failed with status {rc}")
+    return rc == 0
+
+  def conv_wgrad_1x1_nc(self, x: View, tr: Optional[Transform], dy: View, dw: t.Tensor, zero_first: bool = True) -> bool:
+    rc = self.lib._crn_conv_wgrad_1x1_bf3_nc(C.byref(_cview(x)), _ctr(tr), C.byref(_cview(dy)), ptr(dw), int(zero_first),
+                                             _lib.stream())
+    if rc not in (0, -1):
+      raise _lib.HipError(f"crn_conv_wgrad_1x1_bf3_nc failed with status {rc}")
+    return rc == 0
 
   def conv_fwd_stats(self, x: View, tr: Optional[Transform], wslab: t.Tensor, npad: int, bias, bias_sB: int, y: View, window,
                      pad_lo, boxes, Cn: int, pre_relu: bool) -> int:
@@ -382,6 +397,10 @@
   def zero(self, x: t.Tensor):
     self.lib.crn_zero_f32(ptr(x), x.numel(), _lib.stream())
 
+  def zero_ranges(self, base: t.Tensor, table: t.Tensor):
+    if table.shape[0]:
+      self.lib.crn_zero_ranges_f32(ptr(base), ptr(table), table.shape[0], _lib.stream())
+
   def fill_voxels(self, grid: t.Tensor, out: t.Tensor):
     N, D, H, W = grid.shape
     n = self.lib.crn_fill_voxels_workspace_bytes(N, D, H, W)
diff --git a/corenet_amd/csrc/conv_e2d.hip b/corenet_amd/csrc/conv_e2d.hip
--- a/corenet_amd/csrc/conv_e2d.hip
+++ b/corenet_amd/csrc/conv_e2d.hip
@@ -374,12 +374,15 @@
   long long xsB, dsB;
   int C, N, Npad, S;
   int ksteps, ksteps_per_block;
+  int nc;
 };
 
 __global__ __launch_bounds__(256, 2) void wgrad1x1_bf3_kernel(Wg1Geom g) {
   crn_kernargs_now(g.x, g.dy, g.dw, g.scale, g.shift, g.pre_relu, g.post_relu, g.xsB, g.dsB, g.C, g.N, g.Npad, g.S,
-                   g.ksteps, g.ksteps_per_block);
-  __shared__ __attribute__((aligned(16))) f32x4 red[4][8][64];
+                   g.ksteps, g.ksteps_per_block, g.nc);
+  constexpr int kRedPitch = 68;
+  __shared__ __attribute__((aligned(16))) float redf[4 * 32 * kRedPitch];
+  f32x4 (*red)[8][64] = reinterpret_cast<f32x4 (*)[8][64]>(redf);
   const int tid = threadIdx.x, lane = tid & 63;
   const int wave = __builtin_amdgcn_readfirstlane(tid >> 6);
   const int i16 = lane & 15, kk = lane >> 4;
@@ -473,6 +476,23 @@
     }
   }
   wait_all();
+  if (g.nc) {
+#pragma unroll
+    for (int mt = 0; mt < 4; ++mt)
+#pragma unroll
+      for (int nt = 0; nt < 2; ++nt)
+        *reinterpret_cast<f32x4*>(redf + (wave * 32 + 16 * nt + i16) * kRedPitch + 16 * mt + 4 * kk) = acc[mt][nt];
+    __syncthreads();
+    const int c = c0 + lane;
+#pragma unroll
+    for (int q = 0; q < 8; ++q) {
+      const int nl = wave + 4 * q, n = n0 + nl;
+      const float* pr = redf + nl * kRedPitch + lane;
+      const float v = pr[0] + pr[32 * kRedPitch] + pr[2 * 32 * kRedPitch] + pr[3 * 32 * kRedPitch];
+      if (c < g.C && n < g.N) atomicAdd(g.dw + (long long)n * g.C + c, v);
+    }
+    return;
+  }
 #pragma unroll
   for (int mt = 0; mt < 4; ++mt)
 #pragma unroll
@@ -762,15 +782,50 @@
   return crn_conv_wgrad_2d_bf3(x, tr, dy, dw, Npad, 1, 1, 0, 0, zero_first, stream);
 }
 
+namespace {
+bool wg2d_views_ok(const crnView* x, const crnView* dy) {
+  if (!x || !dy || x->B != dy->B || !dense_2d(*x) || !dense_2d(*dy)) return false;
+  if (x->D != dy->D || x->H != dy->H || x->W != dy->W) return false;
+  const int64_t S = (int64_t)x->D * x->H * x->W;
+  if (S % 32 || x->sC != S || dy->sC != S) return false;
+  return S * x->C * 4 < ((int64_t)1 << 31) && S * dy->C * 4 < ((int64_t)1 << 31);
+}
+int wgrad1x1_launch(const crnView* x, const crnInTransform* tr, const crnView* dy, float* dw, int Npad, bool nc,
+                    int zero_first, hipStream_t st) {
+  const int64_t S = (int64_t)x->D * x->H * x->W;
+  if (zero_first) CRN_HIP(hipMemsetAsync(dw, 0, (size_t)x->C * (nc ? dy->C : Npad) * 4, st));
+  Wg1Geom g{};
+  g.x = x->base; g.dy = dy->base; g.dw = dw; g.nc = nc ? 1 : 0;
+  g.scale = tr ? tr->scale : nullptr; g.shift = tr ? tr->shift : nullptr;
+  g.pre_relu = tr ? tr->pre_relu : 0; g.post_relu = tr ? tr->post_relu : 0;
+  g.xsB = x->sB; g.dsB = dy->sB; g.C = x->C; g.N = dy->C; g.Npad = Npad; g.S = (int)S;
+  g.ksteps = (int)((int64_t)x->B * S / 32);
+  const int tiles = crn_cdiv(x->C, 64) * crn_cdiv(dy->C, 32);
+  constexpr int kFill = 512;
+  int splits = std::max(1, std::min(g.ksteps / 8, crn_cdiv(kFill, tiles)));
+  if (crn_deterministic()) splits = 1;
+  g.ksteps_per_block = crn_cdiv(g.ksteps, splits);
+  splits = crn_cdiv(g.ksteps, g.ksteps_per_block);
+  const dim3 grid((unsigned)crn_cdiv(x->C, 64), (unsigned)crn_cdiv(dy->C, 32), (unsigned)splits);
+  hipLaunchKernelGGL(wgrad1x1_bf3_kernel, grid, dim3(256), 0, st, g);
+  CRN_CHECK_LAUNCH();
+  return CRN_OK;
+}
+}
+
+extern "C" int crn_conv_wgrad_1x1_bf3_nc(const crnView* x, const crnInTransform* tr, const crnView* dy, float* dw,
+                                         int zero_first, crnStream stream) {
+  CRN_ENTRY(stream);
+  if (!dw || !wg2d_views_ok(x, dy) || x->C < 1 || dy->C < 1) return CRN_EINVAL;
+  if ((int64_t)x->C * dy->C * 4 >= ((int64_t)1 << 31)) return CRN_EINVAL;
+  return wgrad1x1_launch(x, tr, dy, dw, 0, true, zero_first, (hipStream_t)stream);
+}
+
 extern "C" int crn_conv_wgrad_2d_bf3(const crnView* x, const crnInTransform* tr, const crnView* dy, float* dw, int Npad,
                                      int kh, int kw, int ph, int pw, int zero_first, crnStream stream) {
   CRN_ENTRY(stream);
-  if (!x || !dy || !dw || Npad <= 0 || (Npad & 15) || x->B != dy->B || dy->C > Npad) return CRN_EINVAL;
-  if (!dense_2d(*x) || !dense_2d(*dy)) return CRN_EINVAL;
-  if (x->D != dy->D || x->H != dy->H || x->W != dy->W) return CRN_EINVAL;
+  if (!dw || Npad <= 0 || (Npad & 15) || !wg2d_views_ok(x, dy) || dy->C > Npad) return CRN_EINVAL;
   const int64_t S = (int64_t)x->D * x->H * x->W;
-  if (S % 32 || x->sC != S || dy->sC != S) return CRN_EINVAL;
-  if (S * x->C * 4 >= ((int64_t)1 << 31) || S * dy->C * 4 >= ((int64_t)1 << 31)) return CRN_EINVAL;
   hipStream_t st = (hipStream_t)stream;
   if (kh == 3 && kw == 3) {
     if (ph != 1 || pw != 1 || x->D != 1 || (x->W & 7)) return CRN_EINVAL;
@@ -793,21 +848,5 @@
     return CRN_OK;
   }
   if (kh != 1 || kw != 1 || ph || pw) return CRN_EINVAL;
-  if (zero_first) CRN_HIP(hipMemsetAsync(dw, 0, (size_t)x->C * Npad * 4, st));
-  Wg1Geom g{};
-  g.x = x->base; g.dy = dy->base; g.dw = dw;
-  g.scale = tr ? tr->scale : nullptr; g.shift = tr ? tr->shift : nullptr;
-  g.pre_relu = tr ? tr->pre_relu : 0; g.post_relu = tr ? tr->post_relu : 0;
-  g.xsB = x->sB; g.dsB = dy->sB; g.C = x->C; g.N = dy->C; g.Npad = Npad; g.S = (int)S;
-  g.ksteps = (int)((int64_t)x->B * S / 32);
-  const int tiles = crn_cdiv(x->C, 64) * crn_cdiv(dy->C, 32);
-  constexpr int kFill = 512;
-  int splits = std::max(1, std::min(g.ksteps / 8, crn_cdiv(kFill, tiles)));
-  if (crn_deterministic()) splits = 1;
-  g.ksteps_per_block = crn_cdiv(g.ksteps, splits);
-  splits = crn_cdiv(g.ksteps, g.ksteps_per_block);
-  const dim3 grid((unsigned)crn_cdiv(x->C, 64), (unsigned)crn_cdiv(dy->C, 32), (unsigned)splits);
-  hipLaunchKernelGGL(wgrad1x1_bf3_kernel, grid, dim3(256), 0, st, g);
-  CRN_CHECK_LAUNCH();
-  return CRN_OK;
-}
+  return wgrad1x1_launch(x, tr, dy, dw, Npad, false, zero_first, st);
+}
diff --git a/corenet_amd/csrc/conv_igemm.hip b/corenet_amd/csrc/conv_igemm.hip
--- a/corenet_amd/csrc/conv_igemm.hip
+++ b/corenet_amd/csrc/conv_igemm.hip
@@ -21,12 +21,14 @@
 };
 
 constexpr int kPwTab = 2048;
-template <int NS>
+template <int NS, bool WNC = false>
 __global__ __launch_bounds__(256) void pointwise_fwd_kernel(PwGeom g) {
   constexpr int BM = 64, BN = NS * 16, KC = 64, SA = BM + 16, SB = BN + 16;
+  constexpr int PB = KC + 2;
   constexpr int NRA = KC / 16;
+  typedef float f32x2 __attribute__((ext_vector_type(2)));
   __shared__ __attribute__((aligned(16))) float ldsA[KC * SA];
-  __shared__ __attribute__((aligned(16))) float ldsB[KC * SB];
+  __shared__ __attribute__((aligned(16))) float ldsB[WNC ? BN * PB : KC * SB];
   crn_kernargs_now(g.x, g.y, g.w, g.bias, g.tr.scale, g.tr.shift, g.tr.pre_relu, g.tr.post_relu, g.B, g.C, g.N, g.Npad,
                    g.S, g.xsB, g.ysB, g.ysC, g.ysP, g.bias_sB, g.mode, g.splits, g.cps);
   const long long t_entry = (long long)__builtin_amdgcn_s_memtime();
@@ -43,9 +45,9 @@
   const float* xb = g.x + (int64_t)b * g.xsB;
   const int ka = tid >> 4, ca = (tid & 15) * 4;
   constexpr int BQ = BN / 4, BROWS = 256 / BQ, NRB = KC / BROWS;
-  const int kb = tid / BQ, cb = (tid % BQ) * 4;
+  const int kb = WNC ? tid >> 4 : tid / BQ, cb = WNC ? (tid & 15) * 4 : (tid % BQ) * 4;
   const bool a_ok = (m0 + ca) < g.S;
-  const bool b_ok = (n0 + cb) < g.Npad;
+  const bool b_ok = WNC || (n0 + cb) < g.Npad;
   extern __shared__ float pw_tables[];
   const bool has_tr = g.tr.scale != nullptr;
   float* tsc = pw_tables; float* tsh = pw_tables + g.cps;
@@ -63,8 +65,14 @@
     }
 #pragma unroll
     for (int q = 0; q < NRB; ++q) {
-      const int c_b = c0 + kb + q * BROWS;
-      const unsigned off = (b_ok && c_b < cend) ? (unsigned)(c_b * g.Npad + n0 + cb) * 4u : kOOBo;
+      unsigned off;
+      if constexpr (WNC) {
+        const int n_b = n0 + kb + q * 16, c_b = c0 + cb;
+        off = (n_b < g.N && c_b < cend) ? (unsigned)(n_b * g.C + c_b) * 4u : kOOBo;
+      } else {
+        const int c_b = c0 + kb + q * BROWS;
+        off = (b_ok && c_b < cend) ? (unsigned)(c_b * g.Npad + n0 + cb) * 4u : kOOBo;
+      }
       crnk::crn_bload4(pb_[q], wrs, off);
     }
   };
@@ -103,18 +111,26 @@
 #pragma unroll
     for (int q = 0; q < NRA; ++q) *reinterpret_cast<f32x4*>(ldsA + (ka + q * 16) * SA + ca) = xform(pa_[q], c0 + ka + q * 16);
 #pragma unroll
-    for (int q = 0; q < NRB; ++q) *reinterpret_cast<f32x4*>(ldsB + (kb + q * BROWS) * SB + cb) = pb_[q];
+    for (int q = 0; q < NRB; ++q) {
+      if constexpr (WNC) {
+        float* d = ldsB + (kb + q * 16) * PB + cb;
+        *reinterpret_cast<f32x2*>(d) = (f32x2){pb_[q][0], pb_[q][1]};
+        *reinterpret_cast<f32x2*>(d + 2) = (f32x2){pb_[q][2], pb_[q][3]};
+      } else {
+        *reinterpret_cast<f32x4*>(ldsB + (kb + q * BROWS) * SB + cb) = pb_[q];
+      }
+    }
     __syncthreads();
     mark();
     issue(c0 + 2 * KC, pa_, pb_);
     const float* pa = ldsA + kk * SA + wave * 16 + i16;
-    const float* pb = ldsB + kk * SB + i16;
+    const float* pb = WNC ? ldsB + i16 * PB + kk : ldsB + kk * SB + i16;
 #pragma unroll
     for (int ks = 0; ks < KC / 4; ++ks) {
       const float a = pa[ks * 4 * SA];
       float bv[NS];
 #pragma unroll
-      for (int ns = 0; ns < NS; ++ns) bv[ns] = pb[ks * 4 * SB + ns * 16];
+      for (int ns = 0; ns < NS; ++ns) bv[ns] = WNC ? pb[ks * 4 + ns * 16 * PB] : pb[ks * 4 * SB + ns * 16];
 #pragma unroll
       for (int ns = 0; ns < NS; ++ns) acc[ns] = __builtin_amdgcn_mfma_f32_16x16x4f32(a, bv[ns], acc[ns], 0, 0, 0);
     }
@@ -537,6 +553,68 @@
   return CRN_OK;
 }
 #endif
+static bool pointwise_ok(const crnView* x, const crnInTransform* tr, const float* w, int wrows, int wcols, const crnView* y,
+                         int splits) {
+  const int64_t Sx = (int64_t)x->D * x->H * x->W;
+  return splits <= 1 && plain_view(*x) && flat_out_view(*y) &&
+         Sx == (int64_t)y->D * y->H * y->W && (Sx & 3) == 0 && (((uintptr_t)w) & 15) == 0 &&
+         (int64_t)x->C * Sx * 4 < ((int64_t)1 << 31) && (int64_t)wrows * wcols * 4 < ((int64_t)1 << 31) &&
+         (!tr || !tr->scale || x->C <= kPwTab);
+}
+static int pointwise_launch(const crnView* x, const crnInTransform* tr, const float* w, int Npad, const float* bias,
+                            int bias_sB, const crnView* y, int splits, int accumulate, bool armed, bool w_nc,
+                            hipStream_t st) {
+  const int64_t Sx = (int64_t)x->D * x->H * x->W;
+  PwGeom p{};
+  p.x = x->base; p.y = y->base; p.w = w; p.bias = bias;
+  p.tr = tr ? *tr : crnInTransform{nullptr, nullptr, 0, 0};
+  p.B = x->B; p.C = x->C; p.N = y->C; p.Npad = Npad; p.S = (int)Sx;
+  p.xsB = x->sB; p.ysB = y->sB; p.bias_sB = bias_sB; p.mode = accumulate ? 1 : 0;
+  p.ysC = y->sC; p.ysP = y->sW;
+  p.splits = 1; p.cps = (x->C + 63) & ~63;
+  constexpr int BNh = 32, pw_blocks = 256, pw_fill = 512, pw_minc = 128;
+  const int64_t blocks = crn_cdiv(Sx, 64) * crn_cdiv(y->C, BNh) * (int64_t)x->B;
+  const int64_t ytot = (int64_t)y->B * y->C * Sx;
+  float* scratch = nullptr;
+  if (splits < 1 && blocks < pw_blocks && x->C >= 2 * pw_minc) {
+    int sp = (int)std::min<int64_t>(std::min<int64_t>(x->C / pw_minc, 16), crn_cdiv(pw_fill, blocks));
+    if (sp > 1) {
+      p.cps = (crn_cdiv(x->C, sp) + 31) & ~31;
+      sp = crn_cdiv(x->C, p.cps);
+      if (sp > 1 && (scratch = splitk_scratch((size_t)sp * ytot, st)) != nullptr) {
+        p.splits = sp; p.y = scratch; p.ysB = (int64_t)y->C * Sx; p.ysC = Sx; p.ysP = 1; p.mode = 0;
+      } else {
+        p.cps = (x->C + 31) & ~31;
+      }
+    }
+  }
+#ifdef CRN_TOOLS
+  static const bool want_stamps = getenv("CRN_PW_STAMPS") != nullptr;
+#else
+  constexpr bool want_stamps = false;
+#endif
+  static long long* pw_stamps = nullptr;
+  if (want_stamps) {
+    if (!pw_stamps) CRN_HIP(hipMalloc(&pw_stamps, 32 * sizeof(long long)));
+    CRN_HIP(hipMemsetAsync(pw_stamps, 0, 32 * sizeof(long long), st));
+    p.stamps = pw_stamps;
+    g_pw_stamps = pw_stamps;
+  }
+  dim3 grid((unsigned)crn_cdiv(Sx, 64), (unsigned)crn_cdiv(y->C, BNh), (unsigned)(x->B * p.splits));
+  const size_t tab_bytes = p.tr.scale ? (size_t)2 * p.cps * sizeof(float) : 0;
+  if (w_nc) hipLaunchKernelGGL((pointwise_fwd_kernel<2, true>), grid, dim3(256), tab_bytes, st, p);
+  else hipLaunchKernelGGL((pointwise_fwd_kernel<2, false>), grid, dim3(256), tab_bytes, st, p);
+  CRN_CHECK_LAUNCH();
+  if (p.splits > 1) {
+    if (armed && !accumulate && plain_view(*y) && y->sB == (int64_t)y->C * Sx) {
+      crn_splitk_set_pending(*y, scratch, p.splits, st);
+      return CRN_OK;
+    }
+    return crn_splitk_reduce(*y, scratch, p.splits, accumulate, st);
+  }
+  return CRN_OK;
+}
+
 extern "C" int crn_conv_fwd(const crnView* x, const crnInTransform* tr, const float* w, int Npad,
                             const float* bias, int bias_sB, const crnView* y,
                             int kd, int kh, int kw, int pd, int ph, int pw,
@@ -570,58 +648,8 @@
       return CRN_OK;
     }
   }
-  if (kd * kh * kw == 1 && pd == 0 && ph == 0 && pw == 0 && splits <= 1 && plain_view(*x) && flat_out_view(*y) &&
-      Sx == (int64_t)y->D * y->H * y->W && (Sx & 3) == 0 && (((uintptr_t)w) & 15) == 0 &&
-      (int64_t)x->C * Sx * 4 < ((int64_t)1 << 31) && (int64_t)x->C * Npad * 4 < ((int64_t)1 << 31) &&
-      (!tr || !tr->scale || x->C <= kPwTab)) {
-    PwGeom p{};
-    p.x = x->base; p.y = y->base; p.w = w; p.bias = bias;
-    p.tr = tr ? *tr : crnInTransform{nullptr, nullptr, 0, 0};
-    p.B = x->B; p.C = x->C; p.N = y->C; p.Npad = Npad; p.S = (int)Sx;
-    p.xsB = x->sB; p.ysB = y->sB; p.bias_sB = bias_sB; p.mode = accumulate ? 1 : 0;
-    p.ysC = y->sC; p.ysP = y->sW;
-    p.splits = 1; p.cps = (x->C + 63) & ~63;
-    constexpr int BNh = 32, pw_blocks = 256, pw_fill = 512, pw_minc = 128;
-    const int64_t blocks = crn_cdiv(Sx, 64) * crn_cdiv(y->C, BNh) * (int64_t)x->B;
-    const int64_t ytot = (int64_t)y->B * y->C * Sx;
-    float* scratch = nullptr;
-    if (splits < 1 && blocks < pw_blocks && x->C >= 2 * pw_minc) {
-      int sp = (int)std::min<int64_t>(std::min<int64_t>(x->C / pw_minc, 16), crn_cdiv(pw_fill, blocks));
-      if (sp > 1) {
-        p.cps = (crn_cdiv(x->C, sp) + 31) & ~31;
-        sp = crn_cdiv(x->C, p.cps);
-        if (sp > 1 && (scratch = splitk_scratch((size_t)sp * ytot, st)) != nullptr) {
-          p.splits = sp; p.y = scratch; p.ysB = (int64_t)y->C * Sx; p.ysC = Sx; p.ysP = 1; p.mode = 0;
-        } else {
-          p.cps = (x->C + 31) & ~31;
-        }
-      }
-    }
-#ifdef CRN_TOOLS
-    static const bool want_stamps = getenv("CRN_PW_STAMPS") != nullptr;
-#else
-    constexpr bool want_stamps = false;
-#endif
-    static long long* pw_stamps = nullptr;
-    if (want_stamps) {
-      if (!pw_stamps) CRN_HIP(hipMalloc(&pw_stamps, 32 * sizeof(long long)));
-      CRN_HIP(hipMemsetAsync(pw_stamps, 0, 32 * sizeof(long long), st));
-      p.stamps = pw_stamps;
-      g_pw_stamps = pw_stamps;
-    }
-    dim3 grid((unsigned)crn_cdiv(Sx, 64), (unsigned)crn_cdiv(y->C, BNh), (unsigned)(x->B * p.splits));
-    const size_t tab_bytes = p.tr.scale ? (size_t)2 * p.cps * sizeof(float) : 0;
-    hipLaunchKernelGGL(pointwise_fwd_kernel<2>, grid, dim3(256), tab_bytes, st, p);
-    CRN_CHECK_LAUNCH();
-    if (p.splits > 1) {
-      if (armed && !accumulate && plain_view(*y) && y->sB == (int64_t)y->C * Sx) {
-        crn_splitk_set_pending(*y, scratch, p.splits, st);
-        return CRN_OK;
-      }
-      return crn_splitk_reduce(*y, scratch, p.splits, accumulate, st);
-    }
-    return CRN_OK;
-  }
+  if (kd * kh * kw == 1 && pd == 0 && ph == 0 && pw == 0 && pointwise_ok(x, tr, w, x->C, Npad, y, splits))
+    return pointwise_launch(x, tr, w, Npad, bias, bias_sB, y, splits, accumulate, armed, false, st);
   static const int kM[4] = {8, 4, 2, 1};
   static const int kN[3] = {4, 2, 1};
   const int xmode = vec_view(*x) ? 1 : ((x->sW == 2 && (x->W & 1) == 0) ? 2 : 0);
@@ -861,6 +889,16 @@
 }
 }
 
+extern "C" int crn_conv_fwd_pointwise_nc(const crnView* x, const crnInTransform* tr, const float* w, const float* bias,
+                                         int bias_sB, const crnView* y, int splits, int accumulate, crnStream stream) {
+  if (!x || !y || !w || x->B != y->B || x->B < 1 || x->C < 4 || (x->C & 3) || y->C < 1) return CRN_EINVAL;
+  if (!pointwise_ok(x, tr, w, y->C, x->C, y, splits)) return CRN_EINVAL;
+  hipStream_t st = (hipStream_t)stream;
+  const bool armed = crn_splitk_take_armed();
+  { const int rcf = crn_splitk_flush(st); if (rcf != CRN_OK) return rcf; }
+  return pointwise_launch(x, tr, w, 0, bias, bias_sB, y, splits, accumulate, armed, true, st);
+}
+
 extern "C" int crn_conv_wgrad(const crnView* x, const crnInTransform* tr, const crnView* dy,
                               float* dw, int Npad, int kd, int kh, int kw, int pd, int ph, int pw,
                               int zero_first, const crnTapBoxes* boxes, crnStream stream) {
diff --git a/corenet_amd/csrc/misc_ops.hip b/corenet_amd/csrc/misc_ops.hip
--- a/corenet_amd/csrc/misc_ops.hip
+++ b/corenet_amd/csrc/misc_ops.hip
@@ -477,6 +477,26 @@
   return CRN_OK;
 }
 
+namespace {
+__global__ __launch_bounds__(256) void zero_ranges_kernel(float* base, const long long* tab, long long nrows) {
+  for (long long i = blockIdx.x; i < nrows; i += gridDim.x) {
+    f32x4* p = reinterpret_cast<f32x4*>(base + tab[2 * i]);
+    const long long n4 = tab[2 * i + 1] >> 2;
+    for (long long j = threadIdx.x; j < n4; j += 256) p[j] = (f32x4){0.f, 0.f, 0.f, 0.f};
+  }
+}
+}
+
+extern "C" int crn_zero_ranges_f32(float* base, const int64_t* tab, int64_t nrows, crnStream s) {
+  CRN_ENTRY(s);
+  if (!base || !tab || nrows < 0 || (((uintptr_t)base) & 15)) return CRN_EINVAL;
+  if (nrows == 0) return CRN_OK;
+  hipLaunchKernelGGL(zero_ranges_kernel, dim3((unsigned)std::min<int64_t>(nrows, 16384)), dim3(256), 0, (hipStream_t)s, base,
+                     reinterpret_cast<const long long*>(tab), (long long)nrows);
+  CRN_CHECK_LAUNCH();
+  return CRN_OK;
+}
+
 extern "C" int crn_add_i64(int64_t* p, int n, int64_t v, crnStream s) {
   CRN_ENTRY(s);
   hipLaunchKernelGGL(add_i64_kernel, dim3(nblk(n)), dim3(256), 0, (hipStream_t)s, p, n, v);
diff --git a/corenet_amd/model/engine.py b/corenet_amd/model/engine.py
--- a/corenet_amd/model/engine.py
+++ b/corenet_amd/model/engine.py
@@ -153,6 +153,8 @@
   gwf: t.Tensor
   dbias: t.Tensor
   n_ref: int
+  w_slab: bool = False
+  g_slab: bool = False
   wop_f: Optional[t.Tensor] = None
   wop_d: Optional[t.Tensor] = None
   wop_kind: str = ""
@@ -359,11 +361,23 @@
         p = shape[-1] // 2
         add(name, G.conv_fwd(shape, p), G.conv_dgrad(shape, p))
     idx_parts, sizes = [], []
+    slab_fwd = hasattr(self.be, "conv_fwd_pointwise_nc")
+    slab_grad = slab_fwd and hasattr(self.be, "conv_wgrad_1x1_nc") and self.encoder_e2d
+    self._pw_scratch: Dict[str, tuple] = {}
+    grad_parts, zero_rows = [], []
     for name, fwd, dgrad, repeat, nref in reg:
       wo, bo = s.offset(name + "weight"), s.offset(name + "bias")
       def shift(ix, o):
         return np.where(ix >= 0, ix.astype(np.int64) + o, -1)
       parts = [shift(fwd.index, wo), shift(G.bias_index(nref, repeat, fwd.npad, parity_major=(repeat == 8)), bo)]
+      on_slab = (name.startswith("encoder.stage") and fwd.window == (1, 1, 1) and fwd.cin % 4 == 0 and wo % 4 == 0
+                 and dgrad is not None)
+      grad_parts.append(np.zeros(0, np.int64) if on_slab and slab_grad else parts[0])
+      if on_slab and slab_grad:
+        n = fwd.cin * fwd.nout
+        zero_rows += [(wo + o, min(4096, n - o)) for o in range(0, n, 4096)]
+      if on_slab and slab_fwd:
+        parts[0] = np.zeros(0, np.int64)
       if dgrad is not None:
         alias = (len(dgrad.index) == int(np.prod(s.off[name + "weight"][1]))
                  and np.array_equal(dgrad.index, np.arange(len(dgrad.index))))
@@ -372,17 +386,21 @@
     flat_len = sum(len(p) for parts in idx_parts for p in parts)
     assert max(int(p.max()) for parts in idx_parts for p in parts if len(p)) < 2 ** 31
     self.packed = t.zeros(flat_len, dtype=self.dtype, device=self.device)
-    gsize = sum(len(parts[0]) for parts in idx_parts)
+    gsize = sum(len(gp) for gp in grad_parts)
+    self.gslab_zero = t.as_tensor(np.asarray(zero_rows, np.int64).reshape(-1, 2), device=self.device)
     self.gpacked = t.zeros(gsize, dtype=self.dtype, device=self.device)
     pack_parts, pack_is_bwd, pack_names, unpack_parts = [], [], [], []
     po, go = 0, 0
-    for (name, fwd, dgrad, repeat, nref), parts in zip(reg, idx_parts):
-      pack_parts.append((po, parts[0], fwd.npad, 0)); po += len(parts[0]); pack_is_bwd.append(False); pack_names.append(name)
+    unpack_names = []
+    for (name, fwd, dgrad, repeat, nref), parts, gpart in zip(reg, idx_parts, grad_parts):
+      if len(parts[0]):
+        pack_parts.append((po, parts[0], fwd.npad, 0)); po += len(parts[0]); pack_is_bwd.append(False); pack_names.append(name)
       pack_parts.append((po, parts[1], len(parts[1]), 0)); po += len(parts[1]); pack_is_bwd.append(False); pack_names.append(name)
       if dgrad is not None and len(parts[2]):
         pack_parts.append((po, parts[2], dgrad.npad, dgrad.taps if dgrad.taps > 1 else 0)); po += len(parts[2])
         pack_is_bwd.append(True); pack_names.append(name)
-      unpack_parts.append((go, parts[0], fwd.npad, 0)); go += len(parts[0])
+      if len(gpart):
+        unpack_parts.append((go, gpart, fwd.npad, 0)); go += len(gpart); unpack_names.append(name)
     dev = self._tiles_dev
     self.pack_tiles = dev([pp for pp, bwd in zip(pack_parts, pack_is_bwd) if not bwd])
     sel = lambda pred: [pp for pp, bwd, nm in zip(pack_parts, pack_is_bwd, pack_names) if not bwd and pred(nm)]
@@ -401,14 +419,15 @@
     for lb, lo in zip(GRAD_BUCKET_LABELS, los):
       assert lo < hi
       self.grad_buckets.append((lb, lo, hi))
-      sel = [up for (name, *_), up in zip(reg, unpack_parts) if lo <= s.offset(name + "weight") < hi]
+      sel = [up for name, up in zip(unpack_names, unpack_parts) if lo <= s.offset(name + "weight") < hi]
       self._bucket_tiles.append(sel)
       hi = lo
     self._bucket_dev = None
     po, go = 0, 0
-    for (name, fwd, dgrad, repeat, nref), parts in zip(reg, idx_parts):
+    for (name, fwd, dgrad, repeat, nref), parts, gpart in zip(reg, idx_parts, grad_parts):
       nwf, nb = len(parts[0]), len(parts[1])
-      wf = self.packed[po:po + nwf]; po += nwf
+      w_slab, g_slab = nwf == 0, len(gpart) == 0
+      wf = s.view(name + "weight").view(-1) if w_slab else self.packed[po:po + nwf]; po += nwf
       bias = self.packed[po:po + nb]; po += nb
       wd = None
       if dgrad is not None:
@@ -416,9 +435,9 @@
           wd = self.packed[po:po + len(parts[2])]; po += len(parts[2])
         else:
           wd = s.view(name + "weight").view(-1)
-      gwf = self.gpacked[go:go + nwf]; go += nwf
+      gwf = s.view(name + "weight", grad=True).view(-1) if g_slab else self.gpacked[go:go + len(gpart)]; go += len(gpart)
       self.convs[name] = Conv(name, fwd, dgrad, wf, wd, bias, gwf,
-                              s.view(name + "bias", grad=True), nref)
+                              s.view(name + "bias", grad=True), nref, w_slab=w_slab, g_slab=g_slab)
     self._build_operands(reg, idx_parts)
 
   def _build_ct_images(self):
@@ -499,6 +518,15 @@
     return (t.as_tensor(tl[0], device=self.device), t.as_tensor(tl[1].view(np.int64), device=self.device),
             t.as_tensor(tl[2] if tl[2].size else np.zeros(1, np.int32), device=self.device),
             t.as_tensor(mats, device=self.device))
+
+  def pointwise_scratch(self, cv: Conv):
+    sc = self._pw_scratch.get(cv.name)
+    if sc is None:
+      idx = np.where(cv.fwd.index >= 0, cv.fwd.index.astype(np.int64) + self.store.offset(cv.name + "weight"), -1)
+      sc = (t.zeros(len(idx), dtype=self.dtype, device=self.device), t.zeros(len(idx), dtype=self.dtype, device=self.device),
+            self._tiles_dev([(0, idx, cv.fwd.npad, 0)]))
+      self._pw_scratch[cv.name] = sc
+    return sc
 
   def bucket_unpack_tiles(self, i: int):
     if self._bucket_dev is None:
@@ -770,8 +798,14 @@
       self._timed("fwd   " + cv.name, lambda: self.be.conv2d_bf3(
           x, tr, cv.wop_f, g.npad, cv.bias, 0, y, g.window, g.pad_lo, accumulate))
       return
+    w = cv.wf
+    if cv.w_slab:
+      if self._timed("fwd   " + cv.name, lambda: self.be.conv_fwd_pointwise_nc(x, tr, cv.wf, cv.bias, 0, y, accumulate)):
+        return
+      w, _, tiles = self.eng.pointwise_scratch(cv)
+      self.be.copy_tiles(self.eng.store.params, w, tiles)
     self._timed("fwd   " + cv.name, lambda: self.be.conv_fwd(
-        x, tr, cv.wf, g.npad, cv.bias, 0, y, g.window, g.pad_lo, 0, accumulate, boxes=(g.n_boxes, g.c_boxes),
+        x, tr, w, g.npad, cv.bias, 0, y, g.window, g.pad_lo, 0, accumulate, boxes=(g.n_boxes, g.c_boxes),
         math=self._math(cv, "fwd"), wslab=cv.wop_f if cv.wop_kind == "slab" else None))
 
   def _dgrad(self, cv: Conv, dy: V.View, dx: V.View, accumulate=False):
@@ -815,6 +849,13 @@
   def _launch_wgrad(self, cv: Conv, x: V.View, tr, dy: V.View, math: str, kw: dict):
     g = cv.fwd
     with _lib.roctx_range("wgrad " + cv.name):
+      if cv.g_slab:
+        if math == "bf16x3_2d" and self.be.conv_wgrad_1x1_nc(x, tr, dy, cv.gwf, False):
+          return
+        _, gw, tiles = self.eng.pointwise_scratch(cv)
+        self.be.conv_wgrad(x, tr, dy, gw, g.npad, g.window, g.pad_lo, True, boxes=(g.n_boxes, g.c_boxes), math=math, **kw)
+        self.be.copy_tiles(gw, self.eng.store.grads, tiles, reverse=True)
+        return
       self.be.conv_wgrad(x, tr, dy, cv.gwf, g.npad, g.window, g.pad_lo, False, boxes=(g.n_boxes, g.c_boxes), math=math, **kw)
 
   def _wgrad(self, cv: Conv, x: V.View, tr, dy: V.View, here: bool = False):
@@ -1113,10 +1154,15 @@
     if overlap:
       with self._on_side():
         be.zero(self.gsmap_slab)
+      if eng.gslab_zero.shape[0]:
+        with self._on_side(after=self._next_handover_event()):
+          be.zero_ranges(eng.store.grads, eng.gslab_zero)
       if grad_hook is None:
         grad_hook = _no_exchange
     else:
       be.zero(self.gsmap_slab)
+      if eng.gslab_zero.shape[0]:
+        be.zero_ranges(eng.store.grads, eng.gslab_zero)
     L = eng.latent
     g_out = glogits
     for k in range(6, 1, -1):
diff --git a/include/corenet_hip.h b/include/corenet_hip.h
--- a/include/corenet_hip.h
+++ b/include/corenet_hip.h
@@ -40,6 +40,8 @@
                  int kd, int kh, int kw, int pd, int ph, int pw,
                  int splits, int accumulate ,
                  const crnTapBoxes* boxes , crnStream stream);
+int crn_conv_fwd_pointwise_nc(const crnView* x, const crnInTransform* tr, const float* w, const float* bias, int bias_sB,
+                              const crnView* y, int splits, int accumulate, crnStream stream);
 
 int crn_conv_fwd_bf3(const crnView* x, const crnInTransform* tr, const float* w, int Npad,
                      const float* bias, int bias_sB, const crnView* y,
@@ -95,6 +97,8 @@
 
 int crn_conv_wgrad_1x1_bf3(const crnView* x, const crnInTransform* tr, const crnView* dy, float* dw, int Npad,
                            int zero_first, crnStream stream);
+int crn_conv_wgrad_1x1_bf3_nc(const crnView* x, const crnInTransform* tr, const crnView* dy, float* dw, int zero_first,
+                              crnStream stream);
 int crn_conv_wgrad_2d_bf3(const crnView* x, const crnInTransform* tr, const crnView* dy, float* dw, int Npad,
                           int kh, int kw, int ph, int pw, int zero_first, crnStream stream);
 
@@ -314,6 +318,7 @@
 int crn_set_deterministic(int on);
 
 int crn_zero_f32(float* p, int64_t n, crnStream s);
+int crn_zero_ranges_f32(float* base, const int64_t* tab, int64_t nrows, crnStream s);
 int crn_add_i64(int64_t* p, int n, int64_t v, crnStream s);
 const char* crn_version(void);
 
```

Measured after the change: 1.198 billion (median of 6 runs). No clear change (+0.6%).
